# uf3/uf3

Hardware: AMD Instinct MI355X
Metric: featurized frames/sec (10k-atom, 2-elem, 2+3-body) (higher is better)
Workload: dtype f64

## Files before the change

### include/uf3_hip.h

```cpp
#ifndef UF3_HIP_H
#define UF3_HIP_H

#include <stddef.h>
#include <stdint.h>

#ifdef __cplusplus
extern "C" {
#endif

typedef struct uf3_ctx uf3_ctx;
typedef struct uf3_basis uf3_basis;

enum {
    UF3_OK = 0,
    UF3_EINVAL = 1,
    UF3_ESPECIES = 2,
    UF3_EHIP = 3,
    UF3_ENOMEM = 4,
    UF3_EOVERFLOW = 5,
    UF3_ERETRY = 6
};

typedef struct uf3_basis_spec {
    int32_t n_species;
// ... 35 lines not shown
int uf3_ctx_timing_read(uf3_ctx *ctx, double *featurize_ms, int64_t *featurize_launches,
                        double *neighbor_ms, double *gram_ms, double *eval_ms);

int uf3_ctx_md_skin(uf3_ctx *ctx, double skin);
int uf3_ctx_md_stats(uf3_ctx *ctx, int64_t *builds, int64_t *steps, int64_t *redone);

typedef struct uf3_fit uf3_fit;
int uf3_fit_create(uf3_basis *basis, int with_forces, int64_t max_atoms_per_chunk , const int64_t *frozen_idx,
                   const double *frozen_c, int32_t n_frozen, uf3_fit **out);
void uf3_fit_destroy(uf3_fit *fit);
int uf3_fit_reset(uf3_fit *fit);
int uf3_fit_add(uf3_fit *fit, int32_t n_frames, const int64_t *atom_counts, const double *const *positions, const void *const *z,
                int z_is_int64, const double *cells , const uint8_t *pbc , const double *energies,
                const double *const *forces );
int uf3_fit_pack(uf3_fit *fit, const int64_t *keep, int32_t n_keep, int allreduce, double *out_host);
int uf3_fit_info(const uf3_fit *fit, int64_t *n_chunks, double *n_energy_rows, double *n_force_rows);
int uf3_fit_use_flat(uf3_fit *fit, double *d_flat);
int uf3_fit_first_chunk(uf3_fit *fit, double fraction);

#define UF3_COMM_ID_BYTES 128
int uf3_comm_unique_id(uf3_ctx *ctx, void *id);
int uf3_comm_init(uf3_ctx *ctx, int n_ranks, int rank, const void *id);
int uf3_comm_destroy(uf3_ctx *ctx);
int uf3_comm_info(const uf3_ctx *ctx, int32_t *n_ranks, int32_t *rank);
int uf3_allreduce_sum_f64(uf3_ctx *ctx, double *d_buf, int64_t n);
int uf3_gram_allreduce(uf3_ctx *ctx, double *d_packed, int64_t n);

int uf3_basis_create(uf3_ctx *ctx, const uf3_basis_spec *spec, uf3_basis **out);
void uf3_basis_destroy(uf3_basis *basis);
int uf3_basis_featurizer_modes(const uf3_basis *basis, int32_t *mask);

int uf3_featurize(uf3_basis *basis, const uf3_frames *frames, const double *pos ,
                  const int32_t *z , double *x_e, double *x_f);
int uf3_featurize_dev(uf3_basis *basis, const uf3_frames *frames, const double *d_pos,
                      const int32_t *d_z, double *d_x_e, double *d_x_f);
int uf3_featurize_ld_dev(uf3_basis *basis, const uf3_frames *frames, const double *d_positions, const int32_t *d_z,
                         double *d_x_e, double *d_x_f, int64_t ld);

int uf3_gram(uf3_ctx *ctx, const double *x, const double *y, int64_t n_rows, int32_t n_feat,
             int64_t ld, int accumulate, double *gram, double *ord);
int uf3_gram_dev(uf3_ctx *ctx, const double *d_x, const double *d_y, int64_t n_rows,
                 int32_t n_feat, int64_t ld, int accumulate, double *d_gram, double *d_ord);
int uf3_gram_force_rows_dev(uf3_basis *basis, const double *d_x_f, const double *d_y_f, const int32_t *d_z,
                            int64_t n_atoms, int64_t ld, int accumulate, double *d_gram, double *d_ord);

int uf3_fit_rows_dev(uf3_ctx *ctx, int32_t n_frames, int32_t n_feat, double *d_x_e, const double *d_atom_counts,
                     const double *d_y_e, const double *d_y_f, int64_t n_y_f, const int64_t *d_frozen,
                     const double *d_c_frozen, int32_t n_frozen, double *d_moments );
int uf3_fit_pack_dev(uf3_ctx *ctx, int32_t n_feat, const double *d_flat, const int64_t *d_keep, int32_t n_keep,
                     const int64_t *d_frozen, const double *d_c_frozen, int32_t n_frozen, double n_energy_rows,
                     double n_force_rows, double *d_packed);

int uf3_eval(uf3_basis *basis, const uf3_frames *frames, const double *pos, const int32_t *z,
             const double *c1, const double *c2, const double *c3, double *energies, double *forces);
int uf3_eval_dev(uf3_basis *basis, const uf3_frames *frames, const double *d_pos, const int32_t *d_z,
                 const double *c1, const double *c2, const double *c3 ,
                 double *d_energies, double *d_forces);

int uf3_eval_virial(uf3_basis *basis, const uf3_frames *frames, const double *pos, const int32_t *z,
                    const double *c1, const double *c2, const double *c3, double *energies, double *forces,
                    double *virials);
int uf3_eval_virial_dev(uf3_basis *basis, const uf3_frames *frames, const double *d_pos, const int32_t *d_z,
                        const double *c1, const double *c2, const double *c3 ,
                        double *d_energies, double *d_forces, double *d_virials);

int uf3_eval_atoms(uf3_basis *basis, const uf3_frames *frames, const double *pos, const int32_t *z,
                   const double *c1, const double *c2, const double *c3, int64_t atom_begin, int64_t atom_end,
                   double *energies, double *forces, double *virials);
int uf3_eval_atoms_dev(uf3_basis *basis, const uf3_frames *frames, const double *d_pos, const int32_t *d_z,
                       const double *c1, const double *c2, const double *c3 , int64_t atom_begin,
                       int64_t atom_end, double *d_energies, double *d_forces, double *d_virials);

int uf3_eval_centres(uf3_basis *basis, const uf3_frames *frames, const double *pos, const int32_t *z,
                     const double *c1, const double *c2, const double *c3, int64_t atom_begin, int64_t atom_end,
                     double *energies, double *forces, double *virials);
int uf3_eval_centres_dev(uf3_basis *basis, const uf3_frames *frames, const double *d_pos, const int32_t *d_z,
                         const double *c1, const double *c2, const double *c3 , int64_t atom_begin,
                         int64_t atom_end, double *d_energies, double *d_forces, double *d_virials);

int uf3_neighbors_debug(uf3_basis *basis, const uf3_frames *frame, const double *pos, const int32_t *z,
                        int64_t *pair_count, int64_t *pair_ij, int64_t pair_cap,
                        int64_t *n3_count, int64_t *n3_ij, int64_t n3_cap);
int uf3_n3_lists_debug(uf3_basis *basis, int64_t natoms, int64_t *cap_out, int32_t *counts, int32_t *sidx, int64_t sidx_cap);

int uf3_pair_geometry(uf3_basis *basis, const uf3_frames *frame, const double *pos, const int32_t *z,
                      int64_t *pair_count, int64_t *pair_ij, double *pair_geo, int64_t pair_cap);

int uf3_pair_histogram(uf3_basis *basis, const uf3_frames *frames, const double *pos, const int32_t *z, int32_t n_bins,
                       const double *edges, int upper_inclusive, const double *noise, int64_t n_noise, int per_frame,
                       int64_t *out);
int uf3_pair_histogram_dev(uf3_basis *basis, const uf3_frames *frames, const double *d_pos, const int32_t *d_z, int32_t n_bins,
                           const double *edges, int upper_inclusive, const double *noise, int64_t n_noise, int per_frame,
                           int64_t *d_out);

int uf3_distance_matrix(uf3_ctx *ctx, const double *a, int64_t na, const double *b, int64_t nb, double *out);
int uf3_direction_cosines(uf3_ctx *ctx, const double *sup_pos, int64_t n_sup, const int64_t *i_where,
                          const int64_t *j_where, const double *rij, int64_t n_d, int64_t n_atoms, double *out);

#ifdef __cplusplus
}
#endif
#endif
```

### uf3_amd/_lib.py

```python
import ctypes as C
import sys
import importlib.util
import os
import threading
import weakref

import numpy as np

_HERE = os.path.dirname(os.path.abspath(__file__))
LIB_PATH = os.environ.get("UF3_LIB_PATH", os.path.join(_HERE, "csrc", "libuf3hip.so"))

EXPORTS = ["uf3_ctx_create", "uf3_ctx_destroy", "uf3_ctx_set_stream", "uf3_ctx_synchronize",
           "uf3_last_error", "uf3_build_id", "uf3_ctx_timing_reset", "uf3_ctx_timing_read",
           "uf3_ctx_use_own_stream", "uf3_basis_create", "uf3_basis_destroy", "uf3_basis_featurizer_modes",
           "uf3_featurize", "uf3_featurize_dev", "uf3_gram", "uf3_gram_dev",
           "uf3_eval", "uf3_eval_dev", "uf3_eval_virial", "uf3_eval_virial_dev", "uf3_eval_atoms", "uf3_eval_atoms_dev",
           "uf3_eval_centres", "uf3_eval_centres_dev",
           "uf3_neighbors_debug", "uf3_n3_lists_debug", "uf3_fit_rows_dev", "uf3_fit_pack_dev", "uf3_gram_force_rows_dev",
           "uf3_pair_geometry", "uf3_distance_matrix", "uf3_direction_cosines",
           "uf3_ctx_md_skin", "uf3_ctx_md_stats",
           "uf3_featurize_ld_dev", "uf3_fit_create", "uf3_fit_destroy", "uf3_fit_reset", "uf3_fit_add", "uf3_fit_pack", "uf3_fit_info", "uf3_fit_use_flat", "uf3_fit_first_chunk",
           "uf3_comm_unique_id", "uf3_comm_init", "uf3_comm_destroy", "uf3_comm_info", "uf3_allreduce_sum_f64", "uf3_gram_allreduce",
           "uf3_pair_histogram", "uf3_pair_histogram_dev"]


SOURCES = ("uf3_hip.hip", "uf3_kernels.h", "uf3_feat3.h", "uf3_device.h", os.path.join("..", "..", "include", "uf3_hip.h"))


def source_build_id(csrc_dir=None):
    import hashlib
    csrc_dir = csrc_dir or os.path.join(_HERE, "csrc")
    h = hashlib.sha256()
    for name in SOURCES:
        with open(os.path.join(csrc_dir, name), "rb") as f:
            h.update(f.read())
    return h.hexdigest()[:16]


def build_id():
    return load().uf3_build_id().decode()


class HipUnavailable(RuntimeError):
    pass


class UF3Error(RuntimeError):
    def __init__(self, code, message):
        super().__init__(f"libuf3hip error {code}: {message}")
        self.code = code


class SpeciesError(UF3Error):
    """A frame contains an element outside the basis (UF3_ESPECIES)."""


class RetryError(UF3Error):
    """UF3_ERETRY: an earlier asynchronous ``uf3_featurize_dev`` call overflowed its neighbour capacities (or met atoms
    far outside their cell, whose 3-body force rows need the launches with the reference's image-range rule); its outputs
    are invalid, the context has adapted: repeat the work since the last synchronisation."""


class BasisSpec(C.Structure):
    _fields_ = [("n_species", C.c_int32), ("species_z", C.c_void_p),
                ("n_pairs", C.c_int32), ("pair_z", C.c_void_p), ("pair_nk", C.c_void_p),
                ("pair_knots", C.c_void_p), ("pair_rmin", C.c_void_p), ("pair_rmax", C.c_void_p),
                ("pair_col", C.c_void_p), ("lead2", C.c_int32), ("trail2", C.c_int32),
                ("n_trios", C.c_int32), ("trio_z", C.c_void_p), ("trio_nk", C.c_void_p),
                ("trio_knots", C.c_void_p), ("trio_col", C.c_void_p), ("trio_ncol", C.c_void_p),
                ("trio_lut", C.c_void_p), ("n_feat", C.c_int32), ("r_cut", C.c_double)]


class Frames(C.Structure):
    _fields_ = [("n_frames", C.c_int32), ("atom_offsets", C.c_void_p), ("cells", C.c_void_p),
                ("pbc", C.c_void_p)]


_lib = None
_lock = threading.Lock()


def _share_hip_runtime_with_torch():
    if "torch" in sys.modules:
        return
    try:
        spec = importlib.util.find_spec("torch")
    except (ImportError, ValueError):
        return
    if spec is None or not spec.submodule_search_locations:
        return
    cand = os.path.join(list(spec.submodule_search_locations)[0], "lib", "libamdhip64.so")
    if os.path.exists(cand):
        try:
            C.CDLL(cand, mode=C.RTLD_GLOBAL)
        except OSError:
            pass


def load():
    global _lib
    with _lock:
        if _lib is not None:
            return _lib
        if not os.path.exists(LIB_PATH):
            raise HipUnavailable(
                f"{LIB_PATH} not found: build it with `make -C uf3_amd/csrc` "
                "(or `python -c 'import __graft_entry__ as g; g.build()'`). "
                "uf3_amd has no CPU fallback.")
        _share_hip_runtime_with_torch()
        lib = C.CDLL(LIB_PATH)
        vp, i32, i64, dbl = C.c_void_p, C.c_int32, C.c_int64, C.c_double
        lib.uf3_ctx_create.argtypes = [C.c_int, C.POINTER(vp)]
        lib.uf3_ctx_destroy.argtypes = [vp]
        lib.uf3_ctx_destroy.restype = None
        lib.uf3_ctx_set_stream.argtypes = [vp, vp]
        lib.uf3_ctx_use_own_stream.argtypes = [vp]
        lib.uf3_ctx_synchronize.argtypes = [vp]
        lib.uf3_last_error.argtypes = [vp]
        lib.uf3_last_error.restype = C.c_char_p
        lib.uf3_build_id.argtypes = []
        lib.uf3_build_id.restype = C.c_char_p
        lib.uf3_ctx_timing_reset.argtypes = [vp, C.c_int]
        lib.uf3_ctx_timing_read.argtypes = [vp, C.POINTER(dbl), C.POINTER(i64), C.POINTER(dbl),
                                            C.POINTER(dbl), C.POINTER(dbl)]
        lib.uf3_ctx_md_skin.argtypes = [vp, dbl]
        lib.uf3_fit_create.argtypes = [vp, C.c_int, i64, vp, vp, i32, C.POINTER(vp)]
        lib.uf3_fit_destroy.argtypes = [vp]
        lib.uf3_fit_destroy.restype = None
        lib.uf3_fit_reset.argtypes = [vp]
        lib.uf3_fit_add.argtypes = [vp, i32, vp, vp, vp, C.c_int, vp, vp, vp, vp]
        lib.uf3_fit_pack.argtypes = [vp, vp, i32, C.c_int, vp]
        lib.uf3_fit_info.argtypes = [vp, C.POINTER(i64), C.POINTER(dbl), C.POINTER(dbl)]
        lib.uf3_fit_use_flat.argtypes = [vp, vp]
        lib.uf3_fit_first_chunk.argtypes = [vp, dbl]
        lib.uf3_comm_unique_id.argtypes = [vp, vp]
        lib.uf3_comm_init.argtypes = [vp, C.c_int, C.c_int, vp]
        lib.uf3_comm_destroy.argtypes = [vp]
        lib.uf3_comm_info.argtypes = [vp, C.POINTER(i32), C.POINTER(i32)]
        lib.uf3_allreduce_sum_f64.argtypes = [vp, vp, i64]
        lib.uf3_gram_allreduce.argtypes = [vp, vp, i64]
        lib.uf3_ctx_md_stats.argtypes = [vp, C.POINTER(i64), C.POINTER(i64), C.POINTER(i64)]
        lib.uf3_basis_create.argtypes = [vp, C.POINTER(BasisSpec), C.POINTER(vp)]
        lib.uf3_basis_destroy.argtypes = [vp]
        lib.uf3_basis_destroy.restype = None
        lib.uf3_basis_featurizer_modes.argtypes = [vp, vp]
        for name in ("uf3_featurize", "uf3_featurize_dev"):
            getattr(lib, name).argtypes = [vp, C.POINTER(Frames), vp, vp, vp, vp]
        lib.uf3_featurize_ld_dev.argtypes = [vp, C.POINTER(Frames), vp, vp, vp, vp, i64]
        for name in ("uf3_gram", "uf3_gram_dev"):
            getattr(lib, name).argtypes = [vp, vp, vp, i64, i32, i64, C.c_int, vp, vp]
        for name in ("uf3_eval", "uf3_eval_dev"):
            getattr(lib, name).argtypes = [vp, C.POINTER(Frames), vp, vp, vp, vp, vp, vp, vp]
        for name in ("uf3_eval_virial", "uf3_eval_virial_dev"):
            getattr(lib, name).argtypes = [vp, C.POINTER(Frames), vp, vp, vp, vp, vp, vp, vp, vp]
        for name in ("uf3_eval_atoms", "uf3_eval_atoms_dev", "uf3_eval_centres", "uf3_eval_centres_dev"):
            getattr(lib, name).argtypes = [vp, C.POINTER(Frames), vp, vp, vp, vp, vp, i64, i64, vp, vp, vp]
        lib.uf3_neighbors_debug.argtypes = [vp, C.POINTER(Frames), vp, vp, vp, vp, i64, vp, vp, i64]
        lib.uf3_n3_lists_debug.argtypes = [vp, i64, vp, vp, vp, i64]
        lib.uf3_gram_force_rows_dev.argtypes = [vp, vp, vp, vp, i64, i64, i32, vp, vp]
        lib.uf3_pair_geometry.argtypes = [vp, C.POINTER(Frames), vp, vp, vp, vp, vp, i64]
        lib.uf3_distance_matrix.argtypes = [vp, vp, i64, vp, i64, vp]
        lib.uf3_direction_cosines.argtypes = [vp, vp, i64, vp, vp, vp, i64, i64, vp]
        lib.uf3_fit_rows_dev.argtypes = [vp, i32, i32, vp, vp, vp, vp, i64, vp, vp, i32, vp]
        lib.uf3_fit_pack_dev.argtypes = [vp, i32, vp, vp, i32, vp, vp, i32, dbl, dbl, vp]
        for name in ("uf3_pair_histogram", "uf3_pair_histogram_dev"):
            getattr(lib, name).argtypes = [vp, C.POINTER(Frames), vp, vp, i32, vp, C.c_int, vp, i64, C.c_int, vp]
        _lib = lib
        return lib


def _p(a):
    return None if a is None else a.ctypes.data_as(C.c_void_p)


def _addr(a):
    return None if a is None else a.__array_interface__["data"][0]


class Context:

    def __init__(self, device=0):
        self.lib = load()
        h = C.c_void_p()
        rc = self.lib.uf3_ctx_create(int(device), C.byref(h))
        if rc:
            msg = self.lib.uf3_last_error(None).decode()
            raise HipUnavailable(f"cannot create a HIP context on device {device}: {msg}")
        self.handle = h
        self.device = int(device)
        self._pid = os.getpid()

    def check(self, rc):
        if rc:
            msg = self.lib.uf3_last_error(self.handle).decode()
            raise {2: SpeciesError, 6: RetryError}.get(rc, UF3Error)(rc, msg)

    def set_stream(self, stream_ptr):
        prev = getattr(self, "_stream", None)
        self.check(self.lib.uf3_ctx_set_stream(self.handle, C.c_void_p(stream_ptr or 0)))
        self._stream = stream_ptr or 0
        return prev

    def use_own_stream(self):
        self.check(self.lib.uf3_ctx_use_own_stream(self.handle))
        self._stream = None

    def restore_stream(self, prev):
        if prev is None:
            self.use_own_stream()
        else:
            self.set_stream(prev)

    def synchronize(self):
        self.check(self.lib.uf3_ctx_synchronize(self.handle))

    def timing_reset(self, enable=True):
        self.check(self.lib.uf3_ctx_timing_reset(self.handle, int(enable)))

    def timing_read(self):
        f, n, nb, g, e = C.c_double(), C.c_int64(), C.c_double(), C.c_double(), C.c_double()
        self.check(self.lib.uf3_ctx_timing_read(self.handle, C.byref(f), C.byref(n), C.byref(nb),
                                                C.byref(g), C.byref(e)))
        return dict(featurize_ms=f.value, featurize_launches=n.value, neighbor_ms=nb.value,
                    gram_ms=g.value, eval_ms=e.value)

    def md_skin(self, skin):
        skin = float(skin)
        if getattr(self, "_md_skin", 0.0) != skin:
            self.check(self.lib.uf3_ctx_md_skin(self.handle, skin))
            self._md_skin = skin

    def comm_unique_id(self):
        buf = C.create_string_buffer(128)
        self.check(self.lib.uf3_comm_unique_id(self.handle, buf))
        return buf.raw

    def comm_init(self, n_ranks, rank, unique_id):
        self.check(self.lib.uf3_comm_init(self.handle, int(n_ranks), int(rank), C.c_char_p(bytes(unique_id))))

    def comm_destroy(self):
        self.check(self.lib.uf3_comm_destroy(self.handle))
# ... 269 lines not shown
```

### uf3_amd/csrc/uf3_device.h

```cpp
#pragma once
#include <hip/hip_runtime.h>
#include <stdint.h>
#include <type_traits>

#define UF3_MAX_SPECIES 8
#define UF3_MAX_PAIRS 36
#define WAVE 64

struct KnotRec {
    double t[6];
    double r[6];
};

struct LegDev {
    int rec_off;
    int nk;
    double t0, tlast;
    double inv_h;
};

struct PairDev {
    LegDev leg;
    int col;
    int nb;
// ... 12 lines not shown
    int dim_m, dim_n;
    int dim_l;
    int sc, sa, sb;
    int nsrc, src_off;
    int dense, lo[3], ext[3];
    double thr0, thr2;
    double gthr0, gthr2;
    int grouped;
    int banded;
    int band_tile[3];
    int layout;
    int gsrc_off;
    int wrow[3];
};

struct BasisDev {
    int S, P, T, F;
    int lead2, trail2;
    double rmin3, rmax3;
    double s3_lo, s3_hi;
    double rmax2;
    double rsearch;
    int trio_legs_uniform;
    int pairs_uniform;
    int pair_col[UF3_MAX_SPECIES * UF3_MAX_SPECIES];
    signed char z2s[120];
    short pair_of[UF3_MAX_SPECIES * UF3_MAX_SPECIES];
    short trio_of[UF3_MAX_SPECIES * UF3_MAX_SPECIES * UF3_MAX_SPECIES];
    PairDev pairs[UF3_MAX_PAIRS];
    const TrioDev *trios;
    const KnotRec *recs;
    const int *lut;
};

struct FrameGeom {
    double cell[9];
    double inv[9];
    double binw[3];
    int nb[3];
    int rad[3];
    int per[3];
    int fac[3];
    int cnt[3];
    double win_lo[3], win_hi[3];
    int bin_base;
    int atom_lo, atom_hi;
};

struct __attribute__((aligned(16))) SlotRec {
    double x, y, z;
    int atom;
    int ws;
};
__device__ __forceinline__ int pack_ws(int w0, int w1, int w2, int spec) {
    return (w0 + 256) | ((w1 + 256) << 9) | ((w2 + 256) << 18) | (spec << 27);
}
__device__ __forceinline__ void unpack_ws(int p, int &w0, int &w1, int &w2, int &spec) {
    w0 = (p & 511) - 256; w1 = ((p >> 9) & 511) - 256; w2 = ((p >> 18) & 511) - 256; spec = (p >> 27) & 15;
}

struct CellList {
    const int *bin_start;
    const SlotRec *slots;
    const int *atom_bin;
    const int *atom_wrap;
};

struct __attribute__((aligned(16))) N3Entry {
    double dx, dy, dz, r;
    int parent;
    int shiftc;
    int sidx;
    int spec;
};

struct N3Lists {
    int cap;
    int *cnt;
    int *spoff;
    N3Entry *ent;
    int xcap;
    int *xoff;
    N3Entry *xent;
};

__device__ __forceinline__ int pack3(int a, int b, int c) { return (a + 512) | ((b + 512) << 10) | ((c + 512) << 20); }
__device__ __forceinline__ void unpack3(int p, int &a, int &b, int &c) {
    a = (p & 1023) - 512; b = ((p >> 10) & 1023) - 512; c = ((p >> 20) & 1023) - 512;
}

__device__ __forceinline__ int image_pos(int s) { return s == 0 ? 0 : (s > 0 ? 2 * s - 1 : -2 * s); }

__device__ __forceinline__ int supercell_index(const FrameGeom &g, int s0, int s1, int s2, int local_atom) {
    int rank = (image_pos(s1) * g.cnt[0] + image_pos(s0)) * g.cnt[2] + image_pos(s2);
    return rank * (g.atom_hi - g.atom_lo) + local_atom;
}

__device__ __forceinline__ int find_interval(const KnotRec *recs, const LegDev &leg, double x) {
    int hi = leg.nk - 5;
    int i = 3 + (int)((x - leg.t0) * leg.inv_h);
    i = i < 3 ? 3 : (i > hi ? hi : i);
    const KnotRec *base = recs + leg.rec_off;
    for (;;) {
        double ti = base[i].t[2], ti1 = base[i].t[3];
        if (x > ti1 && i < hi) ++i;
        else if (x <= ti && i > 3) --i;
        else break;
    }
    return i;
}

typedef double __attribute__((ext_vector_type(2))) KnotPair;
template <int AS> struct KnotPairs { typedef const KnotPair *type; };
template <> struct KnotPairs<1> { typedef const __attribute__((address_space(1))) KnotPair *type; };
template <> struct KnotPairs<3> { typedef const __attribute__((address_space(3))) KnotPair *type; };

template <int AS = 0>
__device__ __forceinline__ void load_knot_rec(const KnotRec *p, KnotRec &k) {
    typename KnotPairs<AS>::type q = (typename KnotPairs<AS>::type)(const KnotPair *)p;
    const KnotPair v0 = q[0], v1 = q[1], v2 = q[2], v3 = q[3], v4 = q[4], v5 = q[5];
    __builtin_amdgcn_sched_group_barrier(0x120, 6, 0);
    k.t[0] = v0.x; k.t[1] = v0.y; k.t[2] = v1.x; k.t[3] = v1.y; k.t[4] = v2.x; k.t[5] = v2.y;
    k.r[0] = v3.x; k.r[1] = v3.y; k.r[2] = v4.x; k.r[3] = v4.y; k.r[4] = v5.x; k.r[5] = v5.y;
}

template <int AS = 0>
__device__ __forceinline__ int load_interval(const KnotRec *recs, const LegDev &leg, double x, KnotRec &k) {
    const int hi = leg.nk - 5;
    int i = 3 + (int)((x - leg.t0) * leg.inv_h);
    i = i < 3 ? 3 : (i > hi ? hi : i);
    const KnotRec *base = recs + leg.rec_off;
    load_knot_rec<AS>(base + i, k);
    if (__builtin_expect(x > k.t[3] && i < hi, 0)) {
        do { ++i; load_knot_rec<AS>(base + i, k); } while (x > k.t[3] && i < hi);
    } else if (__builtin_expect(x <= k.t[2] && i > 3, 0)) {
        do { --i; load_knot_rec<AS>(base + i, k); } while (x <= k.t[2] && i > 3);
    }
    return i;
}

template <int AS = 0>
__device__ __forceinline__ int load_interval_guess(const KnotRec *recs, const LegDev &leg, double x, KnotRec &k) {
    const int hi = leg.nk - 5;
    int i = 3 + (int)((x - leg.t0) * leg.inv_h);
    i = i < 3 ? 3 : (i > hi ? hi : i);
    load_knot_rec<AS>(recs + leg.rec_off + i, k);
    return i;
}
template <int AS = 0>
__device__ __forceinline__ int load_interval_fix(const KnotRec *recs, const LegDev &leg, double x, int i, KnotRec &k) {
    const int hi = leg.nk - 5;
    const KnotRec *base = recs + leg.rec_off;
    if (__builtin_expect(x > k.t[3] && i < hi, 0)) {
        do { ++i; load_knot_rec<AS>(base + i, k); } while (x > k.t[3] && i < hi);
    } else if (__builtin_expect(x <= k.t[2] && i > 3, 0)) {
        do { --i; load_knot_rec<AS>(base + i, k); } while (x <= k.t[2] && i > 3);
    }
    return i;
}

template <bool DERIV>
__device__ __forceinline__ void bspline4(const KnotRec &k, double x, double *v, double *d) {
    double l1 = x - k.t[2], l2 = x - k.t[1], l3 = x - k.t[0];
    double r1 = k.t[3] - x, r2 = k.t[4] - x, r3 = k.t[5] - x;
    double tmp = k.r[0];
    double n0 = r1 * tmp, n1 = l1 * tmp;
// ... 63 lines not shown
}
__device__ __forceinline__ int mbcnt(unsigned long long mask) {
    return __builtin_amdgcn_mbcnt_hi((unsigned)(mask >> 32), __builtin_amdgcn_mbcnt_lo((unsigned)mask, 0));
}

template <class F>
__device__ __forceinline__ void for_each_candidate(const FrameGeom &g, const CellList &cl, int m, F f, int range_mult = 1) {
    const int lane = lane_id();
    const int lb = cl.atom_bin[m];
    const int b2 = lb % g.nb[2], b1 = (lb / g.nb[2]) % g.nb[1], b0 = lb / (g.nb[2] * g.nb[1]);
    int w0, w1, w2;
    unpack3(cl.atom_wrap[m], w0, w1, w2);
    int lo[3], hi[3];
    for (int k = 0; k < 3; k++) {
        if (g.per[k]) { lo[k] = -g.rad[k]; hi[k] = g.rad[k]; }
        else if (g.nb[k] == 1) { lo[k] = 0; hi[k] = 0; }
        else if (g.nb[k] == 2) { lo[k] = 0; hi[k] = 1; }
        else { lo[k] = -1; hi[k] = 1; }
    }
    auto fdiv = [](int t, int n) { return t >= 0 ? t / n : -((n - 1 - t) / n); };
    const int n1 = hi[1] - lo[1] + 1, n01 = (hi[0] - lo[0] + 1) * n1;
    const int sh2_lo = fdiv(b2 + lo[2], g.nb[2]), nr2 = fdiv(b2 + hi[2], g.nb[2]) - sh2_lo + 1;
    const int n_runs = n01 * nr2;
    for (int r0 = 0; r0 < n_runs; r0 += WAVE) {
        const int r = r0 + lane;
        int len = 0, slot0 = 0, shp = 0;
        if (r < n_runs) {
            const int i01 = r / nr2, q = r - i01 * nr2, i0 = i01 / n1, i1 = i01 - i0 * n1;
            const int t0 = b0 + lo[0] + i0, t1 = b1 + lo[1] + i1;
            int sh0 = fdiv(t0, g.nb[0]), sh1 = fdiv(t1, g.nb[1]), sh2 = sh2_lo + q;
            const int c0 = t0 - sh0 * g.nb[0], c1 = t1 - sh1 * g.nb[1];
            const int o2a = max(lo[2], sh2 * g.nb[2] - b2), o2b = min(hi[2], (sh2 + 1) * g.nb[2] - 1 - b2);
            const int c2 = b2 + o2a - sh2 * g.nb[2];
            if (!g.per[0]) sh0 = 0;
            if (!g.per[1]) sh1 = 0;
            if (!g.per[2]) sh2 = 0;
            const int gb = g.bin_base + (c0 * g.nb[1] + c1) * g.nb[2] + c2;
            slot0 = cl.bin_start[gb];
            len = cl.bin_start[gb + (o2b - o2a + 1)] - slot0;
            shp = pack3(sh0, sh1, sh2);
        }
        const int incl = wave_scan_incl(len);
        const int total = __builtin_amdgcn_readlane(incl, WAVE - 1);
        const int rel = slot0 - (incl - len);
        const unsigned long long nonempty = __ballot(len > 0);
        const unsigned long long behind = lane < WAVE - 1 ? nonempty >> (lane + 1) : 0ull;
        const int next_ne = behind ? lane + 1 + __builtin_ctzll(behind) : WAVE;
        auto fetch = [&](int wbase, SlotRec &sr, int &shpk) {
            const int idx = wbase + lane;
            const int p = incl - wbase;
            const bool sender = (len > 0) & (p > 0) & (p < WAVE);
            const int got = __builtin_amdgcn_ds_permute((sender ? p : 0) << 2, sender ? next_ne + 1 : 0);
            const unsigned long long holds = __ballot((len > 0) & (p > 0));
            const int first = holds ? __builtin_ctzll(holds) : 0;
            const int reached = wave_scan_max(lane == 0 ? 0 : got);
            const int run = min(reached ? reached - 1 : first, WAVE - 1);
            const int slot = __shfl(rel, run) + idx;
            shpk = __shfl(shp, run);
            sr = cl.slots[idx < total ? slot : 0];
        };
        SlotRec sr_next;
        int shp_next;
        if (total > 0) fetch(0, sr_next, shp_next);
        for (int base = 0; base < total; base += WAVE) {
            const int idx = base + lane;
            SlotRec sr = sr_next;
            const int shpk = shp_next;
            if (base + WAVE < total) fetch(base + WAVE, sr_next, shp_next);
            int sh0, sh1, sh2;
            unpack3(shpk, sh0, sh1, sh2);
            bool ok = idx < total;
            int s0 = 0, s1 = 0, s2 = 0, sj = 0;
            if (ok) {
                int v0, v1, v2;
                unpack_ws(sr.ws, v0, v1, v2, sj);
                s0 = sh0 - v0 + w0; s1 = sh1 - v1 + w1; s2 = sh2 - v2 + w2;
                ok = (abs(s0) <= range_mult * g.fac[0]) && (abs(s1) <= range_mult * g.fac[1]) && (abs(s2) <= range_mult * g.fac[2]);
                if (ok && sr.atom == m && s0 == 0 && s1 == 0 && s2 == 0) ok = false;
            } else { sr.x = sr.y = sr.z = 0.0; sr.atom = 0; sr.ws = 0; }
            f(ok, sr, sj, s0, s1, s2);
        }
    }
}
```

### uf3_amd/csrc/uf3_feat3.h

```cpp
#pragma once

struct Feat3Leg {
    double t0, tlast, inv_h;
    int nk, row0;
};

struct Feat3Args {
    const BasisDev *B;
    const TrioDev *trios;
    const double *rows;
    int n_rows;
    const unsigned short *fsrc;
    const int *trio_fsrc;
    int n_fsrc;
    Feat3Leg leg_p, leg_n;
    int lo_p, ext_p, lo_n, ext_n;
    int pr_rows;
    const FrameGeom *geoms;
    const int *frame_of;
    N3Lists n3;
    const double *pos;
    const signed char *spec;
    double *x_e, *x_f;
    int ld;
    int natoms, atoms_per_block, e_direct;
    const int *sel;
    int sel_mode, sel_cap;
    int skip;
    double *wbuf;
    int wsz;
    int m_lo;
};

template <int EF, int NR>
struct F3Cfg {
    static constexpr int PS = 32 * NR;
    static constexpr int EFP = (EF + 1) & ~1;
    static constexpr int RS_N = EFP + 16 + (NR == 1 ? 2 : 0);
    static constexpr int RS_C = NR == 1 ? 10 : (NR == 2 ? 12 : 14);
    static constexpr int NREC = NR == 1 ? 29 : 32;
    static constexpr int DUMP = NR == 1 ? 4 * EF * 32 : 2 * (EF * PS + 2);
    static constexpr int STAGE0 = 64 * RS_C > NREC * RS_N ? 64 * RS_C : NREC * RS_N;
    static constexpr int STAGE = (STAGE0 > DUMP ? STAGE0 : DUMP) + 4;
    static constexpr int MIN_WAVES = NR == 1 ? 4 : 2;
};

typedef double __attribute__((ext_vector_type(2))) F3Pair;
typedef const __attribute__((address_space(3))) F3Pair *F3LdsPairs;
typedef const __attribute__((address_space(3))) double *F3LdsDoubles;

#ifndef F3_ROWS_GLOBAL
#define F3_ROWS_GLOBAL 0
#endif
typedef const __attribute__((address_space(1))) F3Pair *F3GlobalPairs;
template <bool DERIV>
__device__ __forceinline__ int f3_eval(const double *rows, const Feat3Leg &lg, double x, double (&v)[4], double (&d)[4]) {
    const int hi = lg.nk - 5;
    int iv = 3 + (int)((x - lg.t0) * lg.inv_h);
    iv = iv < 3 ? 3 : (iv > hi ? hi : iv);
    F3Pair kn, cf[8];
    auto load_row = [&](int i) {
#if F3_ROWS_GLOBAL
        F3GlobalPairs q = (F3GlobalPairs)(const F3Pair *)(rows + (size_t)(lg.row0 + i - 3) * 18);
#else
        F3LdsPairs q = (F3LdsPairs)(const F3Pair *)(rows + (size_t)(lg.row0 + i - 3) * 18);
#endif
        F3Pair t0 = q[0], t[8];
#pragma unroll
        for (int e = 0; e < 8; e++) t[e] = q[1 + e];
        kn = t0;
#pragma unroll
        for (int e = 0; e < 8; e++) cf[e] = t[e];
        __builtin_amdgcn_sched_group_barrier(F3_ROWS_GLOBAL ? 0x020 : 0x100, 9, 0);
    };
    load_row(iv);
    if (__builtin_expect(x > kn.y && iv < hi, 0)) {
        do { ++iv; load_row(iv); } while (x > kn.y && iv < hi);
    } else if (__builtin_expect(x <= kn.x && iv > 3, 0)) {
        do { --iv; load_row(iv); } while (x <= kn.x && iv > 3);
    }
    const double u = x - kn.x;
#pragma unroll
    for (int fq = 0; fq < 4; fq++) {
        const double c0 = cf[2 * fq].x, c1 = cf[2 * fq].y, c2 = cf[2 * fq + 1].x, c3 = cf[2 * fq + 1].y;
        double pv = fma(c3, u, c2), pd = fma(c3, u, pv);
        pv = fma(pv, u, c1); pd = fma(pd, u, pv);
        pv = fma(pv, u, c0);
        v[fq] = pv;
        if (DERIV) d[fq] = pd;
    }
    return iv;
}

#ifndef F3_WIDE_MINW
#define F3_WIDE_MINW 2
#endif
template <bool WANT_E, int EF, int NR, int CAP = 0, bool HO = false>
__global__ void __launch_bounds__(WPB * WAVE, (NR == 1 ? 4 : F3_WIDE_MINW))
k_featurize3(Feat3Args A) {
    static_assert(!HO || NR == 1, "the hand-off buffer is laid out for the one-round window");
    typedef F3Cfg<EF, NR> Cfg;
    constexpr int RS_C = Cfg::RS_C, RS_N = Cfg::RS_N, NREC = Cfg::NREC, PS = Cfg::PS, EFP = Cfg::EFP;
    extern __shared__ __align__(16) unsigned char smem[];
    const BasisDev *B = A.B;
    const int F = load_const(&B->F), S = load_const(&B->S), n_trios = load_const(&B->T), cap = CAP > 0 ? CAP : A.n3.cap;
    const int ent_stride = A.n3.cap;
    if (A.sel_mode) {
        const int seen = load_const(A.sel);
        if ((seen <= A.sel_cap) != (A.sel_mode == 1)) return;
    }
    const int tid = threadIdx.x, lane = tid & 63;
    const int wave = __builtin_amdgcn_readfirstlane(tid >> 6);
    double *erow = (double *)smem;
    const bool e_lds = WANT_E && !A.e_direct;
    const size_t e_d = e_lds ? (size_t)F + (F & 1) : 0;
    double *rows_lds = erow + e_d;
    const double *rows = F3_ROWS_GLOBAL ? A.rows : rows_lds;
    const size_t rows_d = (size_t)A.n_rows * 18;
    const size_t list_d = 5 * (size_t)cap + ((5 * cap) & 1), tq_d = (size_t)cap * EF * 4;
    constexpr size_t stage_d = Cfg::STAGE;
    const size_t per_wave_d = list_d + tq_d + stage_d;
    const size_t per_wave_i = 2 * (size_t)cap + 2 * ((size_t)cap + 1) + (UF3_MAX_SPECIES + 2) + (size_t)cap * (S + 1) + 2 * NREC + cap;
    double *wd = rows_lds + rows_d + (size_t)wave * per_wave_d;
    int *wi = (int *)(rows_lds + rows_d + (size_t)WPB * per_wave_d) + (size_t)wave * per_wave_i;
    double *ox = wd, *oy = ox + cap, *oz = oy + cap, *orr = oz + cap, *oir = orr + cap;
    double *tq = wd + list_d;
    double *stage = tq + tq_d;
    double *zq = stage + (Cfg::STAGE - 4);
    int *oparent = wi, *oshift = wi + cap, *noff = wi + 2 * cap, *nbase = noff + cap + 1, *so = nbase + cap + 1;
    int *osbp = so + (UF3_MAX_SPECIES + 2);
    int *hdrs = osbp + cap;
    int *ospoff = hdrs + 2 * NREC;
    const int sp_stride = S + 1;
    unsigned short *fsrc_l = (unsigned short *)((int *)(rows_lds + rows_d + (size_t)WPB * per_wave_d) + (((size_t)WPB * per_wave_i + 3) & ~(size_t)3));

    for (int q = tid; q < (int)rows_d; q += WPB * WAVE) rows_lds[q] = A.rows[q];
    for (int q = tid; q < A.n_fsrc / 2; q += WPB * WAVE) ((int *)fsrc_l)[q] = ((const int *)A.fsrc)[q];
    if (e_lds) { for (int q = tid; q < F; q += WPB * WAVE) erow[q] = 0.0; }
    for (int q = lane; q < (int)stage_d; q += WAVE) stage[q] = 0.0;
    for (int q = lane; q < (int)tq_d; q += WAVE) tq[q] = 0.0;
    __syncthreads();

    const int ext_p = A.ext_p, ext_n = A.ext_n, lo_n = A.lo_n, lo_p = A.lo_p, npos = ext_p * ext_n;
    const int half = lane >> 5;
    int p_lane[NR], n_lane[NR], qn_lane[NR], n32_lane[NR];
    const int pr_rows = A.pr_rows;
#pragma unroll
    for (int r = 0; r < NR; r++) {
        const int pl = (lane & 31) / ext_n, p = r * pr_rows + pl;
        const bool on = pl < pr_rows && p < ext_p;
        p_lane[r] = on ? p : 0;
        n_lane[r] = on ? (lane & 31) - pl * ext_n : -(1 << 20);
        qn_lane[r] = on ? n_lane[r] : RS_C - 1;
        n32_lane[r] = n_lane[r] * 32;
    }
    (void)npos;
    const int sbn_max = ext_n > 4 ? ext_n - 4 : 0, sbp_max = ext_p > 4 ? ext_p - 4 : 0;
    const Feat3Leg leg_p = A.leg_p, leg_n = A.leg_n;
    auto rounds_of = [&](int sb) {
        if (EF <= 4) return (1 << NR) - 1;
        const int r0 = sb / pr_rows, r1 = min(sb + 3, ext_p - 1) / pr_rows;
        return ((2 << r1) - 1) & ~((1 << r0) - 1);
    };

    const int bid = (blockIdx.x & 7) * (gridDim.x >> 3) + (blockIdx.x >> 3);
    const int block_first = A.m_lo + bid * A.atoms_per_block;
    const int block_end = min(block_first + A.atoms_per_block, A.natoms);
    int erow_frame = -1;
    for (int m0 = block_first; m0 < block_end; m0 += WPB) {
        const int m = m0 + wave;
        const bool active = m < block_end;
        if (e_lds) {
            int f_first = load_const(A.frame_of + m0);
            if (f_first != erow_frame) {
                __syncthreads();
                if (erow_frame >= 0)
                    for (int q = tid; q < F; q += WPB * WAVE) {
                        double v = erow[q];
                        if (v != 0.0) { unsafeAtomicAdd(A.x_e + (size_t)erow_frame * F + q, v); erow[q] = 0.0; }
                    }
                __syncthreads();
                erow_frame = f_first;
            }
        }
        if (!active) continue;
        const int fr = load_const(A.frame_of + m);
        const int sm = ((const __attribute__((address_space(4))) signed char *)(unsigned long long)A.spec)[m];
        ESink es;
        es.lds = erow; es.glob = WANT_E ? A.x_e + (size_t)fr * F : nullptr; es.direct = !e_lds || (fr != erow_frame);

        const int n_own = load_const(A.n3.cnt + m);
        wave_sync();
        for (int e = lane; e < n_own; e += WAVE) {
            const N3Entry en = A.n3.ent[(size_t)m * ent_stride + e];
            ox[e] = en.dx; oy[e] = en.dy; oz[e] = en.dz; orr[e] = en.r; oir[e] = 1.0 / en.r;
            int s0, s1, s2;
            unpack3(en.shiftc, s0, s1, s2);
            oparent[e] = en.parent; oshift[e] = pack3(-s0, -s1, -s2);
        }
        if (lane <= S) so[lane] = A.n3.spoff[(size_t)m * (UF3_MAX_SPECIES + 1) + lane];
        wave_sync();
        if (!HO)
            for (int e = lane; e < n_own; e += WAVE) {
                const int *src = A.n3.spoff + (size_t)oparent[e] * (UF3_MAX_SPECIES + 1);
                for (int sp = 0; sp <= S; sp++) ospoff[e * (S + 1) + sp] = src[sp];
            }
        for (int e = lane; e < n_own; e += WAVE) {
            const double r = orr[e];
            double v[4] = {0, 0, 0, 0}, d[4] = {0, 0, 0, 0};
            int sbp = 0;
            if (r > leg_p.t0 && r < leg_p.tlast && !UF3_SKIP(32)) {
                const int iv = f3_eval<true>(rows, leg_p, r, v, d);
                sbp = max(0, min(sbp_max, iv - 3 - lo_p));
            }
            if (EF > 4) osbp[e] = sbp;
            const double ir = oir[e], ux = ox[e] * ir, uy = oy[e] * ir, uz = oz[e] * ir;
            double *dst = tq + (size_t)e * EF * 4;
            if (EF > 4) {
#pragma unroll
                for (int q = 0; q < EF; q++) { *(double2 *)(dst + 4 * q) = double2{0.0, 0.0}; *(double2 *)(dst + 4 * q + 2) = double2{0.0, 0.0}; }
                dst += 4 * sbp;
            }
#pragma unroll
            for (int q = 0; q < (EF < 4 ? EF : 4); q++) {
                *(double2 *)(dst + 4 * q) = double2{ux * d[q], uy * d[q]};
                *(double2 *)(dst + 4 * q + 2) = double2{uz * d[q], v[q]};
            }
        }
        wave_sync();

        for (int t = 0; t < n_trios; t++) {
            const TrioDev *td = A.trios + t;
            typedef int int8_v __attribute__((ext_vector_type(8)));
            const int8_v hv = *(const __attribute__((address_space(4))) int8_v *)(unsigned long long)&td->head;
            const int t_ncol = hv[2], t_sc = hv[3], t_sa = hv[4], t_sb = hv[5], t_col = hv[6];
            const bool centre = t_sc == sm, nbr = t_sa == sm || t_sb == sm;
            if (!centre && !nbr) { zero_rows(A.x_f, m, A.ld, t_col, t_ncol); continue; }
            const bool tr = t_sa != t_sb && sm == t_sb;

            double xacc[NR][EF][2], ws[NR][2];
#pragma unroll
            for (int r = 0; r < NR; r++) {
                ws[r][0] = ws[r][1] = 0.0;
#pragma unroll
                for (int q = 0; q < EF; q++) { xacc[r][q][0] = xacc[r][q][1] = 0.0; }
            }
            int cur = -1;

            int wmask = 0;
            auto flush = [&](bool is_c) {
                if (cur < 0 || UF3_SKIP(2)) return;
                const double *tc = tq + (size_t)cur * EF * 4;
                F3Pair tv[EF];
                double t3[EF];
#pragma unroll
                for (int q = 0; q < EF; q++) {
                    tv[q] = *(F3LdsPairs)(const F3Pair *)(tc + 4 * q + 2 * half); t3[q] = ((F3LdsDoubles)tc)[4 * q + 3];
                }
#pragma unroll
                for (int r = 0; r < NR; r++) {
                    if (EF > 4 && !((wmask >> r) & 1)) continue;
                    const int lo = __double2loint(ws[r][1]), hi = __double2hiint(ws[r][1]);
                    const auto r0 = __builtin_amdgcn_permlane32_swap(lo, lo, false, false);
                    const auto r1 = __builtin_amdgcn_permlane32_swap(hi, hi, false, false);
                    const double wpl = __hiloint2double(r1[1], r0[1]);
                    const double wpl1 = (half && !is_c) ? 0.0 : wpl, ws1 = half ? 0.0 : ws[r][1];
#pragma unroll
                    for (int q = 0; q < EF; q++) {
                        xacc[r][q][0] = fma(tv[q].x, wpl, fma(t3[q], ws[r][0], xacc[r][q][0]));
                        xacc[r][q][1] = fma(tv[q].y, wpl1, fma(t3[q], ws1, xacc[r][q][1]));
                    }
                    ws[r][0] = ws[r][1] = 0.0;
                }
                wmask = 0;
            };

            if (centre && !UF3_SKIP(4)) {
                const int fs = tr ? t_sb : t_sa, gs = tr ? t_sa : t_sb;
                const int f_lo = so[fs], nF = so[fs + 1] - f_lo, g_lo = so[gs], nG = so[gs + 1] - g_lo;
                const bool same = t_sa == t_sb;
                const int total = __builtin_amdgcn_readfirstlane(nF * nG);
                const int nGs = __builtin_amdgcn_readfirstlane(nG), f_los = __builtin_amdgcn_readfirstlane(f_lo),
                          g_los = __builtin_amdgcn_readfirstlane(g_lo);
                const float rcp_ng = __builtin_amdgcn_rcpf((float)max(nG, 1));
                for (int p0 = 0; p0 < total; p0 += WAVE) {
                    const int p = p0 + lane;
                    bool valid = p < total;
                    int fi = (int)(((float)p + 0.5f) * rcp_ng);
                    fi -= (fi * nG > p) ? 1 : 0;
                    fi += ((fi + 1) * nG <= p) ? 1 : 0;
                    const int gi = p - fi * nG;
                    valid = valid && (!same || gi > fi);
                    const int f = f_lo + fi, gg = g_lo + gi;
                    double bn[4] = {0, 0, 0, 0}, dum[4];
                    int sbn = 0;
                    if (valid) {
                        const double rf = orr[f], rg = orr[gg];
                        const double ex = ox[gg] - ox[f], ey = oy[gg] - oy[f], ez = oz[gg] - oz[f];
                        const double rn = norm3_leg(ex, ey, ez);
                        valid = (rf > leg_p.t0) & (rf < leg_p.tlast) & (rg > leg_p.t0) & (rg < leg_p.tlast) &
                                (rn > leg_n.t0) & (rn < leg_n.tlast);
                        if (valid && !UF3_SKIP(64)) {
                            const int iv = f3_eval<false>(rows, leg_n, rn, bn, dum);
                            sbn = max(0, min(sbn_max, iv - 3 - lo_n));
                        }
                    }
                    int smask = (1 << NR) - 1;
                    if (EF > 4) {
                        const int rm = valid ? rounds_of(osbp[gg]) : 0;
                        smask = 0;
#pragma unroll
                        for (int r = 0; r < NR; r++) smask |= __ballot((rm >> r) & 1) ? (1 << r) : 0;
                    }
                    {
                        double *rp = stage + (size_t)lane * RS_C;
#pragma unroll
                        for (int u = 0; u < RS_C; u += 2) *(double2 *)(rp + u) = double2{0.0, 0.0};
                        if (valid) {
#pragma unroll
                            for (int u = 0; u < 4; u++) rp[sbn + u] = bn[u];
                        }
                    }
                    wave_sync();
                    const int p1 = min(total, p0 + WAVE);
                    int fi_s = p0 / nGs;
                    for (int pr = fi_s * nGs; pr < p1 && !UF3_SKIP(1); pr += nGs, fi_s++) {
                        int s0 = max(pr, p0), s1 = min(pr + nGs, p1);
                        if (same) s0 = max(s0, pr + fi_s + 1);
                        if (s0 >= s1) continue;
                        const int key = f_los + fi_s;
                        if (key != cur) { flush(true); cur = key; }
                        wmask |= smask;
                        const double *qp = stage + (size_t)(s0 - p0) * RS_C;
                        const double *tp = tq + (size_t)(g_los + (s0 - pr)) * EF * 4 + 2 * half;
                        int cnt = s1 - s0;
                        auto body = [&](auto tag) {
                            constexpr int CNT = decltype(tag)::value;
#pragma unroll
                            for (int r = 0; r < NR; r++) {
                                if (EF > 4 && !((smask >> r) & 1)) continue;
                                double bq[CNT];
                                F3Pair tt[CNT];
#pragma unroll
                                for (int i = 0; i < CNT; i++) {
                                    bq[i] = ((F3LdsDoubles)qp)[i * RS_C + qn_lane[r]];
                                    tt[i] = *(F3LdsPairs)(const F3Pair *)(tp + (size_t)i * EF * 4 + 4 * p_lane[r]);
                                }
#pragma unroll
                                for (int i = 0; i < CNT; i++) { ws[r][0] = fma(tt[i].x, bq[i], ws[r][0]); ws[r][1] = fma(tt[i].y, bq[i], ws[r][1]); }
                            }
                            qp += CNT * RS_C; tp += (size_t)CNT * EF * 4; cnt -= CNT;
                        };
                        while (cnt >= 4) body(std::integral_constant<int, 4>{});
                        if (cnt == 3) body(std::integral_constant<int, 3>{});
                        else if (cnt == 2) body(std::integral_constant<int, 2>{});
                        else if (cnt == 1) body(std::integral_constant<int, 1>{});
                    }
                    wave_sync();
                }
                flush(true);
                cur = -1;
            }
            if (HO && nbr && !UF3_SKIP(8)) {
                const int sx = sm == t_sa ? t_sb : t_sa;
                const int rc_lo = __builtin_amdgcn_readfirstlane(so[t_sc]), ncen = __builtin_amdgcn_readfirstlane(so[t_sc + 1]) - rc_lo;
                const bool lane_on = n_lane[0] >= 0;
                const size_t wstep = (size_t)S * A.wsz;
                const double *wb = A.wbuf + (((size_t)(m - A.m_lo) * ent_stride + rc_lo) * S + sx) * A.wsz + (lane & 31) * 4 + 2 * half;
                for (int e0 = 0; e0 < ncen; e0 += 4) {
                    F3Pair w[4];
#pragma unroll
                    for (int i = 0; i < 4; i++) {
                        const int idx = min(e0 + i, ncen - 1);
                        w[i] = lane_on ? __builtin_nontemporal_load((const F3Pair *)(wb + (size_t)idx * wstep)) : F3Pair{0.0, 0.0};
                    }
#pragma unroll
                    for (int i = 0; i < 4; i++)
                        if (e0 + i < ncen) {
                            cur = rc_lo + e0 + i;
                            ws[0][0] = w[i].x; ws[0][1] = w[i].y;
                            flush(false);
                        }
                }
                cur = -1;
            }
            if (!HO && nbr && !UF3_SKIP(8)) {
                const int sx = sm == t_sa ? t_sb : t_sa;
                const int rc_lo = so[t_sc], ncen = so[t_sc + 1] - rc_lo;
                int total_n = 0;
                for (int e0 = 0; e0 < ncen; e0 += WAVE) {
                    const int e = e0 + lane;
                    int cnt = 0, base = 0;
                    if (e < ncen) {
                        const int *sp = ospoff + (size_t)(rc_lo + e) * sp_stride;
                        base = sp[sx]; cnt = sp[sx + 1] - base;
                    }
                    const int incl = wave_scan_incl(cnt);
                    if (e < ncen) { noff[e] = total_n + incl - cnt; nbase[e] = base; }
                    total_n += __builtin_amdgcn_readlane(incl, WAVE - 1);
                }
                total_n = __builtin_amdgcn_readfirstlane(total_n);
                if (lane == 0) noff[ncen] = total_n;
                wave_sync();
                for (int p0 = 0; p0 < total_n; p0 += WAVE) {
                    const int q = p0 + lane;
                    bool valid = q < total_n;
                    double pv[4] = {0, 0, 0, 0}, bn[4] = {0, 0, 0, 0}, bd[4] = {0, 0, 0, 0}, a3[3] = {0, 0, 0}, dum[4];
                    int sbn = 0, sbp = 0, e = 0;
                    if (valid) {
                        int lo = 0, hi = ncen - 1;
                        while (lo < hi) { const int mid = (lo + hi + 1) >> 1; if (noff[mid] <= q) lo = mid; else hi = mid - 1; }
                        e = rc_lo + lo;
                        const int kk = nbase[lo] + (q - noff[lo]);
                        const int pc = oparent[e];
                        const double oex = ox[e], oey = oy[e], oez = oz[e], oer = orr[e];
                        const N3Entry ke = A.n3.ent[(size_t)pc * ent_stride + kk];
                        valid = !(ke.parent == m && ke.shiftc == oshift[e]);
                        const double ex = oex + ke.dx, ey = oey + ke.dy, ez = oez + ke.dz;
                        const double rn = norm3_leg(ex, ey, ez), rk = ke.r;
                        valid = valid & (oer > leg_p.t0) & (oer < leg_p.tlast) & (rk > leg_p.t0) & (rk < leg_p.tlast) &
                                (rn > leg_n.t0) & (rn < leg_n.tlast);
                        if (valid && !UF3_SKIP(64)) {
                            const double in = fast_rcp(rn);
                            a3[0] = ex * in; a3[1] = ey * in; a3[2] = ez * in;
                            const int ivp = f3_eval<false>(rows, leg_p, rk, pv, dum);
                            sbp = max(0, min(sbp_max, ivp - 3 - lo_p));
                            const int iv = f3_eval<true>(rows, leg_n, rn, bn, bd);
                            sbn = max(0, min(sbn_max, iv - 3 - lo_n));
                        }
                    }
                    const unsigned long long mask = __ballot(valid);
                    const int nv = __popcll(mask), rank = mbcnt(mask);
                    int smask = (1 << NR) - 1;
                    if (EF > 4) {
                        const int rm = valid ? rounds_of(sbp) : 0;
                        smask = 0;
#pragma unroll
                        for (int r = 0; r < NR; r++) smask |= __ballot((rm >> r) & 1) ? (1 << r) : 0;
                    }
                    for (int sp0 = 0; sp0 < nv; sp0 += NREC) {
                        const int slot = rank - sp0;
                        if (valid && slot >= 0 && slot < NREC) {
                            double *rp = stage + (size_t)slot * RS_N;
                            if (EF > 4) {
#pragma unroll
                                for (int u = 0; u < EFP; u += 2) *(double2 *)(rp + u) = double2{0.0, 0.0};
#pragma unroll
                                for (int u = 0; u < 4; u++) rp[sbp + u] = pv[u];
                            } else {
                                *(double2 *)rp = double2{pv[0], pv[1]};
                                *(double2 *)(rp + 2) = double2{pv[2], pv[3]};
                            }
#pragma unroll
                            for (int u = 0; u < 4; u++) {
                                *(double2 *)(rp + EFP + 4 * u) = double2{a3[0] * bd[u], a3[1] * bd[u]};
                                *(double2 *)(rp + EFP + 2 + 4 * u) = double2{a3[2] * bd[u], bn[u]};
                            }
                            hdrs[slot] = e; hdrs[NREC + slot] = sbn * 32;
                        }
                        wave_sync();
                        const int r_end = min(NREC, nv - sp0);
                        const int v_key = hdrs[min(lane, NREC - 1)], v_prev = hdrs[min(max(lane - 1, 0), NREC - 1)];
                        unsigned long long gm = __ballot(lane < r_end && (lane == 0 || v_key != v_prev));
                        while (gm && !UF3_SKIP(1)) {
                            const int g0 = __builtin_ctzll(gm);
                            gm &= gm - 1;
                            const int g1 = gm ? __builtin_ctzll(gm) : r_end;
                            const int key = __builtin_amdgcn_readlane(v_key, g0);
                            if (key != cur) { flush(false); cur = key; }
                            wmask |= smask;
                            const double *rp = stage + (size_t)g0 * RS_N;
                            const int *sp = hdrs + NREC + g0;
                            int cnt = g1 - g0;
                            auto body = [&](auto tag) {
                                constexpr int CNT = decltype(tag)::value;
                                int sb[CNT];
#pragma unroll
                                for (int i = 0; i < CNT; i++) sb[i] = ((const __attribute__((address_space(3))) int *)sp)[i];
#pragma unroll
                                for (int r = 0; r < NR; r++) {
                                    if (EF > 4 && !((smask >> r) & 1)) continue;
                                    double bq[CNT];
                                    F3Pair tt[CNT];
#pragma unroll
                                    for (int i = 0; i < CNT; i++) {
                                        const unsigned off = (unsigned)(n32_lane[r] - sb[i]);
                                        const char *qa = (const char *)(rp + i * RS_N + EFP + 2 * half) + off;
                                        qa = off < 128u ? qa : (const char *)zq;
                                        bq[i] = ((F3LdsDoubles)rp)[i * RS_N + p_lane[r]];
                                        tt[i] = *(F3LdsPairs)(const F3Pair *)qa;
                                    }
#pragma unroll
                                    for (int i = 0; i < CNT; i++) { ws[r][0] = fma(bq[i], tt[i].x, ws[r][0]); ws[r][1] = fma(bq[i], tt[i].y, ws[r][1]); }
                                }
                                rp += CNT * RS_N; sp += CNT; cnt -= CNT;
                            };
                            while (cnt >= 4) body(std::integral_constant<int, 4>{});
                            if (cnt == 3) body(std::integral_constant<int, 3>{});
                            else if (cnt == 2) body(std::integral_constant<int, 2>{});
                            else if (cnt == 1) body(std::integral_constant<int, 1>{});
                        }
                        wave_sync();
                    }
                }
                flush(false);
                cur = -1;
            }
            if (UF3_SKIP(16)) continue;
            wave_sync();
            const unsigned short *ft = fsrc_l + load_const(A.trio_fsrc + t) + (size_t)(tr ? 2 * t_ncol : 0);
            if (NR == 1) {
#pragma unroll
                for (int q = 0; q < EF; q++)
                    *(double2 *)(stage + (size_t)(((half * EF + q) * 32 + (lane & 31)) * 2)) = double2{xacc[0][q][0], xacc[0][q][1]};
                wave_sync();
                for (int col = lane; col < t_ncol; col += WAVE) {
                    const int s0 = ft[2 * col], s1 = ft[2 * col + 1];
                    F3LdsPairs d0 = (F3LdsPairs)(const F3Pair *)stage, d1 = d0 + EF * 32;
                    const F3Pair a0 = d0[s0], a1 = d0[s1], b0 = d1[s0], b1 = d1[s1];
                    double *dst = A.x_f + (size_t)m * 3 * A.ld + t_col + col;
                    __builtin_nontemporal_store(a0.x + a1.x, dst); __builtin_nontemporal_store(a0.y + a1.y, dst + A.ld);
                    __builtin_nontemporal_store(b0.x + b1.x, dst + 2 * (size_t)A.ld);
                    if (WANT_E) es.add(t_col + col, b0.y + b1.y);
                }
                wave_sync();
            } else {
                constexpr int BUF = EF * PS + 2;
#pragma unroll
                for (int k = 0; k < 2; k++) {
#pragma unroll
                    for (int r = 0; r < NR; r++)
#pragma unroll
                        for (int q = 0; q < EF; q++) stage[half * BUF + q * PS + r * 32 + (lane & 31)] = xacc[r][q][k];
                    if (lane == 0 || lane == 32) stage[half * BUF + EF * PS] = 0.0;
                    wave_sync();
                    for (int col = lane; col < t_ncol; col += WAVE) {
                        const int s0 = ft[2 * col], s1 = ft[2 * col + 1];
                        F3LdsDoubles da = (F3LdsDoubles)stage, db = da + BUF;
                        const double va = da[s0] + da[s1];
                        __builtin_nontemporal_store(va, A.x_f + ((size_t)m * 3 + k) * A.ld + t_col + col);
                        if (k == 0 || WANT_E) {
                            const double vb = db[s0] + db[s1];
                            if (k == 0) __builtin_nontemporal_store(vb, A.x_f + ((size_t)m * 3 + 2) * A.ld + t_col + col);
                            else es.add(t_col + col, vb);
                        }
                    }
                    wave_sync();
                }
            }
        }
    }
    if (e_lds) {
        __syncthreads();
        if (erow_frame >= 0)
            for (int q = tid; q < F; q += WPB * WAVE) {
                double v = erow[q];
                if (v != 0.0) unsafeAtomicAdd(A.x_e + (size_t)erow_frame * F + q, v);
            }
    }
}

#ifndef F3W_NRECP
#define F3W_NRECP 32
#endif
struct F3WCfg {
    static constexpr int RS_W = 38;
    static constexpr int NRECP = F3W_NRECP;
    static constexpr int STAGE = NRECP * RS_W;
};

template <int EF, int CAP = 0>
__global__ void __launch_bounds__(WPB * WAVE, 4)
k_feat3_w(Feat3Args A) {
    static_assert(EF <= 4, "one-round windows only");
    constexpr int RS_W = F3WCfg::RS_W, NRECP = F3WCfg::NRECP;
    extern __shared__ __align__(16) unsigned char smem[];
    const BasisDev *B = A.B;
    const int S = load_const(&B->S), n_trios = load_const(&B->T), cap = CAP > 0 ? CAP : A.n3.cap;
    const int ent_stride = A.n3.cap;
    if (A.sel_mode) {
        const int seen = load_const(A.sel);
        if ((seen <= A.sel_cap) != (A.sel_mode == 1)) return;
    }
    const int tid = threadIdx.x, lane = tid & 63;
    const int wave = __builtin_amdgcn_readfirstlane(tid >> 6);
// ... 165 lines not shown
```

### uf3_amd/csrc/uf3_hip.hip

```cpp
#include <algorithm>
#include <cmath>
#include <cstdio>
#include <cstring>
#include <map>
#include <mutex>
#include <string>
#include <vector>
#include <thread>

#include <hip/hip_runtime.h>
#include <rocprim/rocprim.hpp>

#include "../../include/uf3_hip.h"
#include "uf3_kernels.h"
#include "uf3_feat3.h"
#include <chrono>
#include <dlfcn.h>

struct Buf {
    void *p = nullptr;
    size_t cap = 0;
    bool fine = false;
    hipError_t ensure(size_t bytes) {
        if (bytes <= cap) return hipSuccess;
        if (p) { hipError_t e = hipFree(p); if (e != hipSuccess) return e; p = nullptr; cap = 0; }
        fine = false;
        size_t want = bytes + bytes / 4 + 256;
        hipError_t e = hipMalloc(&p, want);
        if (e == hipSuccess) cap = want;
        return e;
    }
    hipError_t ensure_fine(size_t bytes) {
        if (bytes <= cap && fine) return hipSuccess;
        if (p) { hipError_t e = hipFree(p); if (e != hipSuccess) return e; p = nullptr; cap = 0; }
        fine = false;
        size_t want = std::max(bytes, cap) + bytes / 4 + 256;
        hipError_t e = hipExtMallocWithFlags(&p, want, hipDeviceMallocFinegrained);
        if (e == hipSuccess) { cap = want; fine = true; }
        return e;
    }
    void release() { if (p) hipFree(p); p = nullptr; cap = 0; }
    template <class T> T *as() const { return (T *)p; }
};

struct PinBuf {
    void *p = nullptr;
    size_t cap = 0;
    hipError_t ensure(size_t bytes) {
        if (bytes <= cap) return hipSuccess;
        if (p) hipHostFree(p);
        p = nullptr; cap = 0;
        size_t want = std::max(bytes, (size_t)4096);
        hipError_t e = hipHostMalloc(&p, want, hipHostMallocCoherent);
        if (e == hipSuccess) cap = want;
        return e;
    }
    void release() { if (p) hipHostFree(p); p = nullptr; cap = 0; }
};
#define UF3_PIN_LIMIT (512 * 1024)
#define UF3_BAR_LIMIT (128 * 1024)

struct uf3_ctx {
    int device = 0;
    hipStream_t own_stream = nullptr, stream = nullptr;
    std::string err;
    int lds_max = 65536;
    int n_cu = 256;
    Buf geoms, offsets, frame_of, atom_bin, atom_wrap, spec, key_in, key_out, val_in, val_out, sort_tmp,
        bin_start, slots, flags,
        n3_cnt, n3_int, n3_dbl, e_atom, nbr_f, coeff, stage_pos, stage_z, stage_out, stage_out2,
        gram_tiles[UF3_MAX_SPECIES + 1], gram_tij, frag, dbg,
        sp_rows, sp_seg,
        halo,
        n3x_ent, n3x_off,
        bin_cnt,
        part_sums,
        hist_edges, hist_noise,
        f3w;
    int n3_cap = 0, cand_cap = 0;
    size_t bin_cnt_clean = 0;
    int n3_last_cap = 0, n3_last_natoms = 0;
    int n3x_cap = 0;
    bool img_mode = false;
    int gram_plan_np[UF3_MAX_SPECIES + 1] = {0}, gram_plan_blocks[UF3_MAX_SPECIES + 1] = {0}, gram_plan_next = 0;
    int gram_direct_feat = 0;
    bool n3_tuned = false;
    bool cand_tuned = false;
    struct Pending { hipEvent_t ev = nullptr; int cap = 0, cand = 0, xcap = 0; bool has3 = false, img = true, img_launch = false, live = false; };
    enum { N_PENDING = 16 };
    Pending pending_chk[N_PENDING];
    PinBuf pin_flags;
    int pending_head = 0;
    int async_bad = 0;
    std::string async_msg;
    bool frag_ready = false;
    int32_t *d_stage_z = nullptr;
    bool bar_ok = false;
    bool bar_tested = false;
    Buf stage_bar;
    char *stage_cur = nullptr;
    size_t staged_in_dev = 0;
    bool env_no_feat3 = false, env_f3_no_cap16 = false, env_f3_no_select = false, env_debug_lds = false;
    int env_f3_bps = 24;
    unsigned eval_seq = 0;
    bool tail_signalled = false;
    bool pin_in_busy = false;
    size_t pin_in_pending = 0;
    PinBuf pin_in, pin_geo, pin_out;
    PinBuf pin_eval;
    hipEvent_t pin_in_done = nullptr, pin_geo_done = nullptr;
    std::vector<double> coeff_shadow;
    Buf coeff_cw;
    const void *cw_of = nullptr;
    const void *coeff_dev = nullptr;
    struct MdState {
        bool cap_tuned = false;
        bool verify_next = false;
        bool flags_clean = false;
        double skin = 0.0;
        bool valid = false;
        bool stale = false;
        const uf3_basis *basis = nullptr;
        int natoms = 0, n_frames = 0, cap = 0;
        std::vector<int64_t> offsets;
        std::vector<double> cells;
        std::vector<uint8_t> pbc;
        Buf ent, cnt, pos_ref, geo, frame_of, spec;
        Buf inbox, surv, mark;
        size_t inbox_zeroed = 0;
        size_t geo_bytes = 0;
        long long builds = 0, steps = 0, redone = 0;
    } md;
    void *comm = nullptr;
    int comm_ranks = 0, comm_rank = -1;
    bool md_step = false;
    bool timing = false;
    hipEvent_t ev0 = nullptr, ev1 = nullptr;
    double t_feat = 0, t_nbr = 0, t_gram = 0, t_eval = 0;
    long long n_feat_launch = 0;
    std::vector<std::pair<hipEvent_t, hipEvent_t>> pending[4];
};

struct uf3_basis {
    uf3_ctx *ctx = nullptr;
    BasisDev host;
    BasisDev *dev = nullptr;
    TrioDev *d_trios = nullptr;
    KnotRec *d_recs = nullptr;
    int *d_lut = nullptr;
    int *d_colsrc = nullptr;
    int *d_dsrc = nullptr;
    unsigned short *d_gsrc = nullptr;
    size_t n_gsrc = 0;
    bool all_grouped7 = false;
    bool all_banded9 = false;
    size_t n_dsrc = 0;
    int *d_sp_cols = nullptr;
    int sp_ncols[UF3_MAX_SPECIES] = {0};
    std::vector<int> block_bounds;
    size_t c2_len = 0, c3_len = 0, n_recs = 0;
    size_t n_pair_recs = 0;
    size_t trio_rec_lo = 0;
    size_t wrow_lo = 0;
    int n_wrows = 0;
// ... 34 lines not shown
        if (eq) g_env.vars.emplace_back(std::string(*e, eq - *e), std::string(eq + 1));
    }
}
static const char *uf3_env(const char *name) {
    if (g_env.print == ~0ull) uf3_env_refresh();
    for (const auto &kv : g_env.vars)
        if (kv.first == name) return kv.second.c_str();
    return nullptr;
}

static inline void uf3_store_fence() {
#if defined(__x86_64__) || defined(__i386__)
    __builtin_ia32_sfence();
#else
    __sync_synchronize();
#endif
}

static thread_local std::string g_err;
static int fail(uf3_ctx *ctx, int code, const std::string &msg) {
    if (ctx) ctx->err = msg;
    g_err = msg;
    return code;
}
#define HIPCHK(ctx, call)                                                                         \
    do {                                                                                          \
        hipError_t e__ = (call);                                                                  \
        if (e__ != hipSuccess)                                                                    \
            return fail(ctx, UF3_EHIP, std::string(#call) + ": " + hipGetErrorString(e__));       \
    } while (0)

extern "C" const char *uf3_last_error(const uf3_ctx *ctx) { return ctx ? ctx->err.c_str() : g_err.c_str(); }
#ifndef UF3_BUILD_ID
#define UF3_BUILD_ID "unknown"
#endif
extern "C" const char *uf3_build_id(void) { return UF3_BUILD_ID; }

static void read_f3_env(uf3_ctx *c) {
    c->env_no_feat3 = uf3_env("UF3_NO_FEAT3") != nullptr;
    c->env_f3_no_cap16 = uf3_env("UF3_F3_NO_CAP16") != nullptr;
    c->env_f3_no_select = uf3_env("UF3_F3_NO_SELECT") != nullptr;
    c->env_debug_lds = uf3_env("UF3_DEBUG_LDS") != nullptr;
    c->env_f3_bps = uf3_env("UF3_F3_BPS") ? std::max(1, atoi(uf3_env("UF3_F3_BPS"))) : 24;
}

extern "C" int uf3_ctx_create(int device, uf3_ctx **out) {
    uf3_env_refresh();
    if (!out) return fail(nullptr, UF3_EINVAL, "uf3_ctx_create: null out");
    int n = 0;
    hipError_t e = hipGetDeviceCount(&n);
    if (e != hipSuccess || n <= 0)
        return fail(nullptr, UF3_EHIP, std::string("no HIP device available: ") + hipGetErrorString(e));
    if (device < 0 || device >= n) return fail(nullptr, UF3_EINVAL, "uf3_ctx_create: bad device index");
    uf3_ctx *c = new uf3_ctx();
    c->device = device;
    HIPCHK(c, hipSetDevice(device));
    HIPCHK(c, hipStreamCreateWithFlags(&c->own_stream, hipStreamNonBlocking));
    c->stream = c->own_stream;
    HIPCHK(c, hipEventCreateWithFlags(&c->pin_in_done, hipEventDisableTiming));
    HIPCHK(c, hipEventCreateWithFlags(&c->pin_geo_done, hipEventDisableTiming));
    hipDeviceProp_t prop;
    HIPCHK(c, hipGetDeviceProperties(&prop, device));
    c->lds_max = (int)prop.sharedMemPerBlock;
    c->n_cu = prop.multiProcessorCount;
    read_f3_env(c);
    { int large = 0; c->bar_ok = hipDeviceGetAttribute(&large, hipDeviceAttributeIsLargeBar, device) == hipSuccess && large && !uf3_env("UF3_NO_BAR_STAGE"); }
    if (std::string(prop.gcnArchName).find("gfx950") == std::string::npos) {
        std::string m = std::string("uf3_hip is built for gfx950 only, device is ") + prop.gcnArchName;
        delete c;
        return fail(nullptr, UF3_EHIP, m);
    }
    *out = c;
    return UF3_OK;
}

extern "C" int uf3_comm_destroy(uf3_ctx *c);
extern "C" void uf3_ctx_destroy(uf3_ctx *c) {
    if (!c) return;
    hipSetDevice(c->device);
    hipStreamSynchronize(c->stream);
    Buf *all[] = {&c->geoms, &c->offsets, &c->frame_of, &c->atom_bin, &c->atom_wrap, &c->spec, &c->key_in,
                  &c->key_out, &c->val_in, &c->val_out, &c->sort_tmp, &c->bin_start, &c->slots, &c->flags, &c->n3_cnt, &c->n3_int, &c->n3_dbl, &c->e_atom, &c->nbr_f, &c->coeff,
                  &c->stage_pos, &c->stage_z, &c->stage_out, &c->stage_out2, &c->sp_rows, &c->sp_seg, &c->gram_tij, &c->frag, &c->dbg, &c->halo, &c->n3x_ent, &c->n3x_off,
                  &c->bin_cnt, &c->f3w, &c->coeff_cw, &c->part_sums};
    for (Buf *b : all) b->release();
    for (Buf &b : c->gram_tiles) b.release();
    if (c->comm) uf3_comm_destroy(c);
    { Buf *mdb[] = {&c->md.ent, &c->md.cnt, &c->md.pos_ref, &c->md.geo, &c->md.frame_of, &c->md.spec, &c->md.inbox, &c->md.surv, &c->md.mark}; for (Buf *b : mdb) b->release(); }
    c->stage_bar.release();
    c->pin_in.release(); c->pin_geo.release(); c->pin_out.release(); c->pin_flags.release(); c->pin_eval.release();
    for (auto &pd : c->pending_chk) if (pd.ev) hipEventDestroy(pd.ev);
    if (c->pin_in_done) hipEventDestroy(c->pin_in_done);
    if (c->pin_geo_done) hipEventDestroy(c->pin_geo_done);
    for (auto &v : c->pending) for (auto &p : v) { hipEventDestroy(p.first); hipEventDestroy(p.second); }
    if (c->own_stream) hipStreamDestroy(c->own_stream);
    delete c;
}

extern "C" int uf3_ctx_set_stream(uf3_ctx *c, void *s) {
    if (!c) return fail(nullptr, UF3_EINVAL, "null ctx");
    c->stream = (hipStream_t)s;
    return UF3_OK;
}

extern "C" int uf3_ctx_use_own_stream(uf3_ctx *c) {
    if (!c) return fail(nullptr, UF3_EINVAL, "null ctx");
    c->stream = c->own_stream;
    return UF3_OK;
}

static int check_flags(uf3_ctx *c);
static int poll_pending(uf3_ctx *c, bool wait, bool remember = true);

extern "C" int uf3_ctx_synchronize(uf3_ctx *c) {
    if (!c) return fail(nullptr, UF3_EINVAL, "null ctx");
    HIPCHK(c, hipSetDevice(c->device));
    HIPCHK(c, hipStreamSynchronize(c->stream));
    poll_pending(c, true);
    if (c->async_bad) {
        const int rc = c->async_bad;
        const std::string msg = c->async_msg;
        c->async_bad = 0; c->async_msg.clear();
        return fail(c, rc, msg);
    }
    return check_flags(c);
}

static int sync_own_call(uf3_ctx *c) {
    HIPCHK(c, hipStreamSynchronize(c->stream));
    int rc = poll_pending(c, true, false);
    if (rc) return rc;
    return check_flags(c);
}

enum { T_FEAT = 0, T_NBR = 1, T_GRAM = 2, T_EVAL = 3 };
struct Timed {
    uf3_ctx *c; int cls; hipEvent_t a = nullptr, b = nullptr;
    Timed(uf3_ctx *c_, int cls_) : c(c_), cls(cls_) {
        if (c->timing) { hipEventCreate(&a); hipEventCreate(&b); hipEventRecord(a, c->stream); }
    }
    ~Timed() {
        if (c->timing) { hipEventRecord(b, c->stream); c->pending[cls].push_back({a, b}); if (cls == T_FEAT) c->n_feat_launch++; }
    }
};

extern "C" int uf3_ctx_timing_reset(uf3_ctx *c, int enable) {
    if (!c) return fail(nullptr, UF3_EINVAL, "null ctx");
    hipStreamSynchronize(c->stream);
    for (auto &v : c->pending) { for (auto &p : v) { hipEventDestroy(p.first); hipEventDestroy(p.second); } v.clear(); }
    c->t_feat = c->t_nbr = c->t_gram = c->t_eval = 0;
    c->n_feat_launch = 0;
    c->timing = enable != 0;
    return UF3_OK;
}

extern "C" int uf3_ctx_timing_read(uf3_ctx *c, double *feat_ms, int64_t *feat_launches, double *nbr_ms,
                                   double *gram_ms, double *eval_ms) {
    if (!c) return fail(nullptr, UF3_EINVAL, "null ctx");
    HIPCHK(c, hipStreamSynchronize(c->stream));
    double *acc[4] = {&c->t_feat, &c->t_nbr, &c->t_gram, &c->t_eval};
    for (int k = 0; k < 4; k++) {
        for (auto &p : c->pending[k]) {
            float ms = 0;
            hipEventElapsedTime(&ms, p.first, p.second);
            *acc[k] += ms;
            hipEventDestroy(p.first); hipEventDestroy(p.second);
        }
// ... 622 lines not shown
    for (int k = 0; k < 3; k++) {
        double h = vol / norm3(nrm[k]);
        g.cnt[k] = g.per[k] ? 2 * g.fac[k] + 1 : 1;
        if (g.per[k]) {
            int nb = (int)std::floor(h / (rs * bin_frac));
            nb = std::max(1, std::min(nb, 256));
            g.nb[k] = nb;
            g.rad[k] = (int)std::ceil(rs / (h / nb) - 1e-12);
            if (g.rad[k] < 1) g.rad[k] = 1;
            g.binw[k] = 1.0 / nb;
            if (g.fac[k] > 400) return fail(c, UF3_EINVAL, "cell is too small relative to the cutoff");
            const double w = g.fac[k] + 1.0 - b->r_cut / h - 1e-9;
            g.win_lo[k] = 0.5 - 0.5 * w; g.win_hi[k] = 0.5 + 0.5 * w;
        } else {
            g.win_lo[k] = -1e300; g.win_hi[k] = 1e300;
            g.nb[k] = nb_np;
            g.rad[k] = 1;
            g.binw[k] = rs / h;
        }
        nbins *= g.nb[k];
    }
    long long m = (long long)g.cnt[0] * g.cnt[1] * g.cnt[2] * n;
    if (m >= (1LL << 31)) return fail(c, UF3_EINVAL, "reference supercell index exceeds int32");
    g.bin_base = bin_cursor;
    if (nbins + bin_cursor >= (1LL << 30)) return fail(c, UF3_EINVAL, "too many cell-list bins");
    bin_cursor += (int)nbins;
    return UF3_OK;
}

struct Prepared {
    int natoms = 0, n_frames = 0, nbins = 0;
    double max_density = 0;
    CellList cl;
    N3Lists n3;
    const FrameGeom *geoms = nullptr;
    const int *frame_of = nullptr;
    const signed char *spec = nullptr;
    const int64_t *d_offsets = nullptr;
    size_t geo_bytes = 0;
    bool deferred = false;
    bool flags_zeroed = false;
    bool small_prepared = false;
};

static int check_flags(uf3_ctx *c) {
    if (!c->flags.p) return UF3_OK;
    int fl[4] = {0, 0, 0, 0};
    HIPCHK(c, hipMemcpy(fl, c->flags.p, sizeof(fl), hipMemcpyDeviceToHost));
    if (fl[0] == 2) { hipMemset(c->flags.p, 0, sizeof(fl)); return fail(c, UF3_ESPECIES, "frame contains an element outside the basis"); }
    if (fl[0] == 1) { hipMemset(c->flags.p, 0, sizeof(fl)); return fail(c, UF3_EINVAL, "atom too far outside the periodic cell (|wrap| > 250)"); }
    return UF3_OK;
}

static int poll_pending(uf3_ctx *c, bool wait, bool remember) {
    int rc = UF3_OK;
    for (int q = 0; q < uf3_ctx::N_PENDING; q++) {
        uf3_ctx::Pending &p = c->pending_chk[(c->pending_head + q) % uf3_ctx::N_PENDING];
        if (!p.live) continue;
        if (wait) { HIPCHK(c, hipEventSynchronize(p.ev)); }
        else if (hipEventQuery(p.ev) != hipSuccess) continue;
        p.live = false;
        const int *fl = (const int *)c->pin_flags.p + 8 * ((c->pending_head + q) % uf3_ctx::N_PENDING);
        if (fl[0] == 2 && !rc) rc = fail(c, UF3_ESPECIES, "frame contains an element outside the basis (earlier asynchronous call)");
        else if (fl[0] == 1 && !rc) rc = fail(c, UF3_EINVAL, "atom too far outside the periodic cell (|wrap| > 250) (earlier asynchronous call)");
        bool grown = false;
        if (p.has3 && fl[1] > p.cap) { c->n3_cap = std::max(c->n3_cap, (std::max(fl[1] + 8, p.cap + p.cap / 4) + 7) / 8 * 8); grown = true; }
        if (fl[2] > p.cand) { c->cand_cap = std::max(c->cand_cap, (std::max(fl[2] + 16, p.cand + p.cand / 4) + 7) / 8 * 8); grown = true; }
        if (fl[3] > p.xcap) { c->n3x_cap = std::max(c->n3x_cap, std::min(248, (fl[3] + 8 + 7) / 8 * 8)); grown = true; }
        if (fl[4] && !p.img) { c->img_mode = true; grown = true; }
        else if (!fl[4] && p.img_launch) c->img_mode = false;
        if (grown && !rc)
            rc = fail(c, UF3_ERETRY, "an earlier asynchronous featurizer call overflowed its neighbour capacities: its outputs are "
                                     "invalid; the capacities have been raised, repeat the work since the last synchronisation");
    }
    if (rc && c->flags.p) hipMemsetAsync(c->flags.p, 0, sizeof(int), c->stream);
    if (rc && remember && !c->async_bad) { c->async_bad = rc; c->async_msg = c->err; }
    return rc;
}

static int n3_alloc(uf3_ctx *c, int natoms, int cap, N3Lists &n3) {
    HIPCHK(c, c->n3_cnt.ensure(sizeof(int) * (size_t)natoms * (UF3_MAX_SPECIES + 2)));
    HIPCHK(c, c->n3_dbl.ensure(sizeof(N3Entry) * (size_t)natoms * cap));
    n3.cap = cap;
    c->n3_last_cap = cap; c->n3_last_natoms = natoms;
    n3.cnt = c->n3_cnt.as<int>();
    n3.spoff = n3.cnt + natoms;
    n3.ent = c->n3_dbl.as<N3Entry>();
    return UF3_OK;
}

static int n3_cap_estimate(const uf3_basis *b, double dens) {
    double r = b->host.rmax3;
    double est = dens > 0 ? 4.18879 * r * r * r * dens : 24.0;
    return std::max(16, ((int)(est * 1.8) + 8 + 7) / 8 * 8);
}

static int n3_tune(uf3_ctx *c, const N3Lists &n3, int natoms) {
    hipStream_t st = c->stream;
    int *flags = c->flags.as<int>();
    c->n3_tuned = true;
    HIPCHK(c, hipMemsetAsync(flags + 6, 0, sizeof(int), st));
    hipLaunchKernelGGL(k_max_count, dim3(64), dim3(256), 0, st, n3.cnt, natoms, flags + 6);
    int seen = 0;
    HIPCHK(c, hipMemcpyAsync(&seen, flags + 6, sizeof(int), hipMemcpyDeviceToHost, st));
    HIPCHK(c, hipStreamSynchronize(st));
    c->n3_cap = std::max(8, (seen + 7) / 8 * 8);
    return UF3_OK;
}

static int build_halo_lists(uf3_basis *b, const Prepared &P, const N3Lists &n3, const double *d_pos, int lo, int hi,
                            bool marks_zeroed = false) {
    uf3_ctx *c = b->ctx;
    hipStream_t st = c->stream;
    const int natoms = P.natoms, nb_ = hi - lo;
    HIPCHK(c, c->halo.ensure(sizeof(int) * ((size_t)natoms + 4)));
    int *mark = c->halo.as<int>(), *range = mark + natoms;
    if (!marks_zeroed) HIPCHK(c, hipMemsetAsync(mark, 0, sizeof(int) * (size_t)natoms, st));
    if (nb_ <= 0 || natoms - nb_ <= 0) return UF3_OK;
    const size_t lds = (size_t)n3.cap * (8 + 32 + 16);
    hipLaunchKernelGGL(k_mark_halo, dim3((nb_ + 3) / 4), dim3(256), 0, st, n3, lo, hi, mark, range);
    hipLaunchKernelGGL(k_build_n3, dim3(natoms - nb_), dim3(64), lds, st, b->dev, P.geoms, P.frame_of, P.cl, n3, d_pos,
                       natoms, c->flags.as<int>() + 1, 0, (const int *)mark, (const int *)range);
    HIPCHK(c, hipGetLastError());
    return UF3_OK;
}

static int prepare(uf3_basis *b, const uf3_frames *fr, const double *d_pos, const int32_t *d_z, bool need_n3,
                   Prepared &P, bool defer_check = false, int64_t n3_lo = 0, int64_t n3_hi = -1, double extra_radius = 0.0) {
    uf3_ctx *c = b->ctx;
    c->md.flags_clean = false;
    if (!fr || fr->n_frames < 1 || !fr->atom_offsets || !fr->cells || !fr->pbc)
        return fail(c, UF3_EINVAL, "bad uf3_frames");
    if (fr->atom_offsets[0] != 0) return fail(c, UF3_EINVAL, "atom_offsets[0] must be 0");
    int nf = fr->n_frames;
    int64_t total = fr->atom_offsets[nf];
    if (total < 1 || total >= (1LL << 31) / 8) return fail(c, UF3_EINVAL, "batch must hold 1 .. 2^28 atoms");
    for (int f = 0; f < nf; f++)
        if (fr->atom_offsets[f + 1] < fr->atom_offsets[f]) return fail(c, UF3_EINVAL, "atom_offsets must be non-decreasing");
    int natoms = (int)total;
    std::vector<FrameGeom> geoms(nf);
    int bin_cursor = 0;
    double dens = 0;
    for (int f = 0; f < nf; f++) {
        int rc = make_geom(c, b, fr, f, geoms[f], bin_cursor, extra_radius);
        if (rc) return rc;
        int n = geoms[f].atom_hi - geoms[f].atom_lo;
        double vol = 0;
        if (geoms[f].per[0] && geoms[f].per[1] && geoms[f].per[2]) {
            double cr[3];
            cross3(geoms[f].cell + 3, geoms[f].cell + 6, cr);
            vol = std::fabs(dot3(geoms[f].cell, cr));
        }
        if (vol > 0) dens = std::max(dens, n / vol);
    }
    int nbins = bin_cursor;
    hipStream_t st = c->stream;
    HIPCHK(c, hipSetDevice(c->device));
    const size_t geo_bytes = (sizeof(FrameGeom) * nf + 15) / 16 * 16, off_bytes = sizeof(int64_t) * (nf + 1);
    const FrameGeom *d_geoms;
    const int64_t *d_offsets;
    const int4 *host_block = nullptr;
    size_t host_block_bytes = 0;
    if (c->staged_in_dev && d_pos == (const double *)c->stage_cur) {
        const size_t at = c->staged_in_dev;
        c->staged_in_dev = 0;
        std::memcpy(c->stage_cur + at, geoms.data(), sizeof(FrameGeom) * nf);
        std::memcpy(c->stage_cur + at + geo_bytes, fr->atom_offsets, off_bytes);
// ... 79 lines not shown
    P.geo_bytes = geo_bytes + off_bytes;
    P.geoms = d_geoms;
    P.frame_of = c->frame_of.as<int>();
    P.spec = c->spec.as<signed char>();
    P.d_offsets = d_offsets;
    P.cl.bin_start = c->bin_start.as<int>(); P.cl.slots = c->slots.as<SlotRec>();
    P.cl.atom_bin = c->atom_bin.as<int>(); P.cl.atom_wrap = c->atom_wrap.as<int>();
    std::memset(&P.n3, 0, sizeof(P.n3));
    if (need_n3 && b->host.T > 0) {
        if (c->n3_cap == 0) c->n3_cap = n3_cap_estimate(b, dens);
        for (int attempt = 0; attempt < 6; attempt++) {
            int cap = c->n3_cap;
            int rc = n3_alloc(c, natoms, cap, P.n3);
            if (rc) return rc;
            HIPCHK(c, hipMemsetAsync(flags + 1, 0, sizeof(int), st));
            size_t lds = (size_t)cap * (8 + 32 + 16);
            if ((int)lds > c->lds_max) return fail(c, UF3_EOVERFLOW, "3-body neighbour list does not fit in LDS");
            const bool block_only = n3_hi >= 0 && !(n3_lo == 0 && n3_hi == natoms) && !uf3_env("UF3_NO_HALO");
            if (!block_only)
                hipLaunchKernelGGL(k_build_n3, dim3(natoms), dim3(64), lds, st, b->dev, P.geoms, P.frame_of, P.cl, P.n3,
                                   d_pos, natoms, flags + 1, 0, (const int *)nullptr, (const int *)nullptr);
            else if (n3_hi > n3_lo) {
                const int nb_ = (int)(n3_hi - n3_lo);
                HIPCHK(c, hipMemsetAsync(P.n3.cnt, 0, sizeof(int) * (size_t)natoms, st));
                hipLaunchKernelGGL(k_build_n3, dim3(nb_), dim3(64), lds, st, b->dev, P.geoms, P.frame_of, P.cl, P.n3,
                                   d_pos, natoms, flags + 1, (int)n3_lo, (const int *)nullptr, (const int *)nullptr);
                int rh = build_halo_lists(b, P, P.n3, d_pos, (int)n3_lo, (int)n3_hi);
                if (rh) return rh;
            }
            HIPCHK(c, hipGetLastError());
            if (defer_check && c->n3_tuned) { P.deferred = true; return UF3_OK; }
            int fl[4] = {0, 0, 0, 0};
            HIPCHK(c, hipMemcpyAsync(fl, flags, sizeof(fl), hipMemcpyDeviceToHost, st));
            HIPCHK(c, hipStreamSynchronize(st));
            if (fl[0]) return check_flags(c);
            const int need = fl[1];
            if (need <= cap) {
                if (!c->n3_tuned) { int rt = n3_tune(c, P.n3, natoms); if (rt) return rt; }
                return UF3_OK;
            }
            c->n3_tuned = true;
            c->n3_cap = (need + 8 + 7) / 8 * 8;
        }
        return fail(c, UF3_EOVERFLOW, "3-body neighbour capacity did not converge");
    }
    return UF3_OK;
}

static int ensure_frag(uf3_ctx *c);

static size_t feat_lds_bytes(int F, int S, int cap, int cand_cap, bool want_e, size_t n_recs, int mode, int dense_stage,
                             int dense_nrec, int n_pair_cols) {
    const bool dense = mode >= 6;
    if (mode == 0) F = S + n_pair_cols;
    size_t e_d = want_e ? (size_t)F + (F & 1) : 0;
    size_t cand_d = (size_t)cand_cap * CAND_STRIDE;
    size_t pair_buf_d = std::max(4 * (size_t)n_pair_cols, (3 * (size_t)cap + 1) / 2 + 2);
    size_t stage_d = mode == 0 ? cand_d + pair_buf_d
                     : (dense ? (size_t)dense_stage : (size_t)NSTAGE * ITEM_STRIDE);
    size_t list_d = mode == 0 ? 0 : 5 * (size_t)cap + ((5 * cap) & 1);
    size_t geo_d = dense ? (size_t)7 * GEO_N : 0;
    size_t per_wave_d = list_d + stage_d + (stage_d & 1) + geo_d;
    size_t per_wave_i = mode == 0 ? 0 : 3 * (size_t)cap + 2 * ((size_t)cap + 1) + (UF3_MAX_SPECIES + 2) +
                                        (size_t)cap * (S + 1);
    size_t ints = ((size_t)WPB * per_wave_i + 3) & ~(size_t)3;
    return (e_d + WPB * per_wave_d) * 8 + ints * 4 + n_recs * sizeof(KnotRec) + 32;
}

static void feat3_shape(const uf3_basis *b, int &ep, int &stage, int &nrec) {
    ep = std::max(3, b->f3_ext_p);
    switch (ep) {
        case 3: stage = F3Cfg<3, 1>::STAGE; nrec = F3Cfg<3, 1>::NREC; break;
        case 4: stage = F3Cfg<4, 2>::STAGE; nrec = F3Cfg<4, 2>::NREC; break;
        case 5: stage = F3Cfg<5, 3>::STAGE; nrec = F3Cfg<5, 3>::NREC; break;
        default: stage = F3Cfg<6, 3>::STAGE; nrec = F3Cfg<6, 3>::NREC; break;
    }
}
static size_t feat3_lds_bytes(const uf3_basis *b, int cap, bool e_lds) {
    int ep, stage, nrec;
    feat3_shape(b, ep, stage, nrec);
    const int F = b->host.F, S = b->host.S;
    const size_t e_d = e_lds ? (size_t)F + (F & 1) : 0, rows_d = (size_t)b->n_f3rows * 18;
    const size_t list_d = 5 * (size_t)cap + ((5 * cap) & 1), tq_d = (size_t)cap * ep * 4, stage_d = (size_t)stage;
    const size_t per_wave_i = 2 * (size_t)cap + 2 * ((size_t)cap + 1) + (UF3_MAX_SPECIES + 2) + (size_t)cap * (S + 1) + 2 * (size_t)nrec + (size_t)cap;
    const size_t ints = ((size_t)WPB * per_wave_i + 3) & ~(size_t)3;
    return (e_d + rows_d + WPB * (list_d + tq_d + stage_d)) * 8 + ints * 4 + (size_t)b->n_f3src * 2 + 32;
}
static size_t feat3w_lds_bytes(const uf3_basis *b, int cap) {
    const size_t rows_d = (size_t)b->n_f3rows * 18;
    const size_t per_wave_d = 8 * (size_t)cap + F3WCfg::STAGE, per_wave_i = 4 * (size_t)cap + (UF3_MAX_SPECIES + 2);
    return (rows_d + WPB * per_wave_d) * 8 + WPB * per_wave_i * 4 + 32;
}
#define UF3_LDS_LIMIT ((size_t)160 * 1024 - 512)

static int featurize_dev_impl(uf3_basis *b, const uf3_frames *fr, const double *d_pos, const int32_t *d_z,
                              double *d_xe, double *d_xf, int64_t ld);

extern "C" int uf3_featurize_dev(uf3_basis *b, const uf3_frames *fr, const double *d_pos, const int32_t *d_z,
                                 double *d_xe, double *d_xf) {
    if (!b) return fail(nullptr, UF3_EINVAL, "null basis");
    return featurize_dev_impl(b, fr, d_pos, d_z, d_xe, d_xf, b->host.F);
}

extern "C" int uf3_featurize_ld_dev(uf3_basis *b, const uf3_frames *fr, const double *d_pos, const int32_t *d_z,
                                    double *d_xe, double *d_xf, int64_t ld) {
    if (!b) return fail(nullptr, UF3_EINVAL, "null basis");
    if (ld < b->host.F || ld > (1 << 24)) return fail(b->ctx, UF3_EINVAL, "uf3_featurize_ld_dev: ld must be >= the number of features");
    return featurize_dev_impl(b, fr, d_pos, d_z, d_xe, d_xf, ld);
}

static int featurize_dev_impl(uf3_basis *b, const uf3_frames *fr, const double *d_pos, const int32_t *d_z,
                              double *d_xe, double *d_xf, int64_t ld) {
    uf3_ctx *c = b->ctx;
    uf3_env_refresh();
    read_f3_env(c);
    if (!d_pos || !d_z) return fail(c, UF3_EINVAL, "null positions / species");
    if (!d_xe && !d_xf) return UF3_OK;
    { int rc0 = poll_pending(c, false, false); if (rc0) return rc0; }
    Prepared P;
    const bool old_n3 = uf3_env("UF3_SEPARATE_N3") != nullptr;
    int rc = prepare(b, fr, d_pos, d_z, old_n3, P);
    if (rc) return rc;
    hipStream_t st = c->stream;
    const int F = b->host.F;
    const bool want_e = d_xe != nullptr, want_f = d_xf != nullptr;
    const bool has3 = b->host.T > 0 && !old_n3;
    if (has3 && c->n3_cap == 0) c->n3_cap = n3_cap_estimate(b, P.max_density);
    int cap = 1;
    auto cand_estimate = [&]() {
        double r = b->host.rsearch;
        double est = P.max_density > 0 ? 4.18879 * r * r * r * P.max_density : 64.0;
        return std::max(32, ((int)(est * 1.6) + 16 + 7) / 8 * 8);
    };
    if (c->cand_cap == 0) c->cand_cap = cand_estimate();
    bool caps_reset = false;
    FeatArgs A;
    A.B = b->dev; A.trios = b->d_trios; A.recs = b->d_recs; A.colsrc = b->d_colsrc;
    A.frag = nullptr;
    A.dense_stage = 0; A.dense_nrec = DENSE_NREC;
    A.dsrc = b->d_dsrc; A.n_dsrc = (int)b->n_dsrc;
    A.gsrc = b->d_gsrc; A.n_gsrc = (int)b->n_gsrc; A.gsrc_lds = 0;
    const int dense_modes = (1 << 6) | (1 << 7) | (1 << 8) | (1 << 9);
    const bool dsrc_ok = (b->modes & dense_modes) && b->n_dsrc * sizeof(int) <= 8192 && !uf3_env("UF3_NO_LDS_DSRC");
    A.dsrc_lds = dsrc_ok;
    if (b->modes & dense_modes) { rc = ensure_frag(c); if (rc) return rc; A.frag = c->frag.as<int>(); }
    A.geoms = P.geoms; A.frame_of = P.frame_of; A.cl = P.cl;
    std::memset(&A.n3, 0, sizeof(A.n3));
    A.n3.cap = 1;
    if (old_n3 && P.n3.cap) A.n3 = P.n3;
    A.build_n3 = has3 ? 1 : 0;
    A.e_direct = (want_e && (size_t)F * 8 > 48 * 1024) ? 1 : 0;
    A.n3_need = c->flags.as<int>() + 1;
    A.n3_seen = nullptr;
    A.pos = d_pos; A.spec = P.spec; A.x_e = d_xe; A.x_f = d_xf; A.ld = (int)ld; A.natoms = P.natoms;
    A.cand_need = c->flags.as<int>() + 2;
    A.outside = uf3_env("UF3_KEEP_GHOST_TERMS") ? nullptr : c->flags.as<int>() + 4;
    { const char *e = uf3_env("UF3_DEBUG_SKIP"); A.skip = e ? atoi(e) : 0; }
    for (int attempt = 0; attempt < 6; attempt++) {
        A.cand_cap = c->cand_cap;
        A.n_recs = (int)b->n_recs;
        A.n_pair_recs = (int)b->n_pair_recs;
        A.trio_rec_lo = (int)b->trio_rec_lo;
        A.wrow_base = (int)(b->wrow_lo * 6); A.n_wrows = b->n_wrows;
        A.n_pair_cols = 0;
        for (int p = 0; p < b->host.P; p++) A.n_pair_cols += b->host.pairs[p].nb;
        if (old_n3) cap = A.n3.cap;
        if (has3) {
            cap = c->n3_cap;
            rc = n3_alloc(c, P.natoms, cap, A.n3);
            if (rc) return rc;
        }
        if (want_e) HIPCHK(c, hipMemsetAsync(d_xe, 0, sizeof(double) * (size_t)P.n_frames * F, st));
        if (!P.flags_zeroed || attempt) HIPCHK(c, hipMemsetAsync(A.n3_need, 0, 2 * sizeof(int), st));
        const bool img_launch = c->img_mode && has3 && want_f && A.outside;
        const bool ext_lists = img_launch;
        if (ext_lists) {
            const int xcap = c->n3x_cap;
            A.n3.xcap = xcap; A.n3.xent = nullptr; A.n3.xoff = nullptr;
            if (xcap > 0) {
                HIPCHK(c, c->n3x_ent.ensure(sizeof(N3Entry) * (size_t)P.natoms * xcap));
                HIPCHK(c, c->n3x_off.ensure(sizeof(int) * (size_t)P.natoms * (UF3_MAX_SPECIES + 1)));
                A.n3.xent = c->n3x_ent.as<N3Entry>(); A.n3.xoff = c->n3x_off.as<int>();
            }
            hipLaunchKernelGGL(k_build_n3_ext, dim3(std::min(P.natoms, 2048)), dim3(64), (size_t)xcap * (8 + 32 + 12) + 16, st,
                               b->dev, P.geoms, P.frame_of, P.cl, A.n3, d_pos, P.natoms, c->flags.as<int>());
        }
        const bool feat3 = b->feat3_ok && want_f && (has3 || old_n3) && !img_launch && cap <= 255 && !c->env_no_feat3 &&
                           feat3_lds_bytes(b, cap, want_e && !A.e_direct) <= UF3_LDS_LIMIT;
        A.n3_seen = nullptr;
        if (feat3 && has3 && cap > 16 && !c->env_f3_no_cap16 && !c->env_f3_no_select) {
            A.n3_seen = c->flags.as<int>() + 7;
            HIPCHK(c, hipMemsetAsync(A.n3_seen, 0, sizeof(int), st));
        }
        bool restart = false;
        {
            Timed tm(c, T_FEAT);
            for (int mode = 0; mode <= 9; mode++) {
                if (!(b->modes & (1 << mode))) continue;
                if (feat3 && mode >= 1) continue;
                const bool dense_mode = mode >= 6;
                const int launch_mode = (mode == 7 && want_f && b->all_grouped7 && !img_launch && !uf3_env("UF3_NO_GROUPED_ONLY")) ? 10
                                        : ((mode == 9 && want_f && b->all_banded9 && !img_launch && !uf3_env("UF3_NO_GROUPED_ONLY")) ? 11 : mode);
                A.trio_rec_lo = (int)(launch_mode == 10 ? b->wrow_lo : b->trio_rec_lo);
                size_t n_rec_mode = mode == 0 ? b->n_pair_recs : b->n_recs - (size_t)A.trio_rec_lo;
                const int S = b->host.S;
                const size_t cu_lds = 160 * 1024 - 1024;
                if (dense_mode) A.dsrc_lds = dsrc_ok && !(mode == 7 && want_f && b->all_grouped7);
                const bool gsrc_wanted = mode == 7 && want_f && b->dense_grouped[7] && b->n_gsrc > 0 && b->n_gsrc * 2 <= 4096 && !uf3_env("UF3_NO_LDS_GSRC");
                const size_t gsrc_bytes = gsrc_wanted ? b->n_gsrc * 2 : 0;
                A.gsrc_lds = gsrc_wanted;
                size_t lds_extra = ((dense_mode && A.dsrc_lds) ? sizeof(int) * b->n_dsrc : 0) + gsrc_bytes;
                bool recs_lds = false;
                size_t lds = 0, lds_plain = 0, lds_recs = 0;
                bool found = false;
                if (dense_mode) {
                    const int stride = want_f ? b->dense_stride_f[mode] : b->dense_stride[mode];
                    const int dump = want_f && b->dense_grouped[mode] ? std::max(768, b->dense_dump[mode]) : b->dense_dump[mode];
                    const bool grouped = want_f && b->dense_grouped[mode];
                    const int nrec_max = std::max(4, std::min(DENSE_NREC, 1200 / stride));
                    auto stage_for = [&](int nr) { return std::max(dump, (nr + (nr & 1) + (grouped ? 2 : 0)) * stride); };
                    A.dense_nrec = nrec_max; A.dense_stage = stage_for(nrec_max);
                    if (mode <= 7 && !uf3_env("UF3_NO_OCC3")) {
                        const int tries[3] = {nrec_max, std::min(nrec_max, 20), std::min(nrec_max, 15)};
                        const size_t budget = (WPB == 4 ? 52 : 13 * WPB) * 1024;
                        const bool dsrc_allowed = A.dsrc_lds, recs_allowed = !uf3_env("UF3_NO_LDS_RECS") && !(img_launch && mode != 0);
                        for (int q = 0; q < 12 && !found; q++) {
                            const int nr = tries[(q % 6) / 2];
                            const bool with_recs = q < 6, with_dsrc = (q & 1) == 0;
                            if ((with_recs && !recs_allowed) || (with_dsrc && !dsrc_allowed)) continue;
                            size_t need = feat_lds_bytes(F, S, cap, A.cand_cap, want_e && !A.e_direct, with_recs ? n_rec_mode : 0, mode,
                                                         stage_for(nr), nr, A.n_pair_cols) + (with_dsrc ? sizeof(int) * b->n_dsrc : 0) + gsrc_bytes;
                            if (need <= budget) {
                                found = true; recs_lds = with_recs; lds = lds_recs = need;
                                A.dense_nrec = nr; A.dense_stage = stage_for(nr); A.dsrc_lds = with_dsrc;
                            }
                        }
                    }
                }
                if (!found) {
                    lds_plain = feat_lds_bytes(F, S, cap, A.cand_cap, want_e && !A.e_direct, 0, mode, A.dense_stage, A.dense_nrec, A.n_pair_cols) + lds_extra;
                    lds_recs = feat_lds_bytes(F, S, cap, A.cand_cap, want_e && !A.e_direct, n_rec_mode, mode, A.dense_stage, A.dense_nrec, A.n_pair_cols) + lds_extra;
                    const size_t lds_target = cu_lds / (mode == 0 ? 4 : 2);
                    recs_lds = lds_recs <= lds_target && !uf3_env("UF3_NO_LDS_RECS") && !(img_launch && mode != 0);
                    lds = recs_lds ? lds_recs : lds_plain;
                }
                if (lds > UF3_LDS_LIMIT && mode == 0 && !c->cand_tuned && c->cand_cap > 64) {
                    while (c->cand_cap > 64 && feat_lds_bytes(F, S, cap, c->cand_cap, want_e && !A.e_direct, recs_lds ? n_rec_mode : 0, 0,
                                                              A.dense_stage, A.dense_nrec, A.n_pair_cols) + lds_extra > UF3_LDS_LIMIT)
                        c->cand_cap = (c->cand_cap * 7 / 8 + 7) / 8 * 8;
                    A.cand_cap = c->cand_cap;
                    lds = feat_lds_bytes(F, S, cap, A.cand_cap, want_e && !A.e_direct, recs_lds ? n_rec_mode : 0, 0, A.dense_stage,
                                         A.dense_nrec, A.n_pair_cols) + lds_extra;
                }
                if (lds > UF3_LDS_LIMIT && !caps_reset) {
                    const int est3 = has3 ? n3_cap_estimate(b, P.max_density) : 0, estc = cand_estimate();
                    if ((has3 && c->n3_cap > est3) || c->cand_cap > estc) {
                        if (has3 && c->n3_cap > est3) { c->n3_cap = est3; c->n3_tuned = false; }
                        if (c->cand_cap > estc) { c->cand_cap = estc; c->cand_tuned = false; }
                        caps_reset = restart = true;
                        break;
                    }
                }
                if (lds > UF3_LDS_LIMIT) return fail(c, UF3_EOVERFLOW, "featurizer LDS footprint exceeds 160 KB (F or neighbour count too large)");
                int per_cu = std::max(1, std::min(8, (int)((size_t)(160 * 1024) / lds)));
                int n_blocks = std::min((P.natoms + WPB - 1) / WPB, c->n_cu * per_cu * 24);
                int apb = ((P.natoms + n_blocks - 1) / n_blocks + WPB - 1) / WPB * WPB;
                n_blocks = (P.natoms + apb - 1) / apb;
                A.atoms_per_block = apb;
                if (uf3_env("UF3_DEBUG_LDS"))
                    fprintf(stderr, "uf3 featurize mode %d: lds %zu B (plain %zu, with recs %zu), recs_lds %d, cap %d, cand_cap %d, "
                            "blocks %d x %d atoms, n_recs %zu, dense nrec %d stage %d\n", launch_mode, lds, lds_plain, lds_recs,
                            (int)recs_lds, cap, A.cand_cap, n_blocks, apb, n_rec_mode, A.dense_nrec, A.dense_stage);
#define UF3_GRID(n) (((n) + 7) / 8 * 8)
 \
#define UF3_LAUNCH1(E, Fo, R, M, I)                                                                                   \
    do {                                                                                                            \
        {                                                                                                           \
            static std::mutex mu; static size_t have[64] = {0};                                                     \
            std::lock_guard<std::mutex> lk(mu);                                                                     \
            size_t &hv = have[c->device & 63];                                                                      \
            if (lds > hv) {                                                                                         \
                HIPCHK(c, hipFuncSetAttribute((const void *)k_featurize<E, Fo, R, M, I>, hipFuncAttributeMaxDynamicSharedMemorySize, (int)lds)); \
                hv = lds;                                                                                           \
            }                                                                                                       \
        }                                                                                                           \
        hipLaunchKernelGGL((k_featurize<E, Fo, R, M, I>), dim3(UF3_GRID(n_blocks)), dim3(WPB * WAVE), lds, st, A);   \
    } while (0)
#define UF3_LAUNCH(M)                                                                                               \
    do {                                                                                                            \
        if (img_launch && M != 0) {          \
            if (want_e) UF3_LAUNCH1(true, true, false, (M == 0 ? 1 : M), true); else UF3_LAUNCH1(false, true, false, (M == 0 ? 1 : M), true); \
        }                                                                                                           \
        else if (want_e && want_f) { if (recs_lds) UF3_LAUNCH1(true, true, true, M, false); else UF3_LAUNCH1(true, true, false, M, false); }   \
        else if (want_f) { if (recs_lds) UF3_LAUNCH1(false, true, true, M, false); else UF3_LAUNCH1(false, true, false, M, false); }    \
        else { if (recs_lds) UF3_LAUNCH1(true, false, true, M, false); else UF3_LAUNCH1(true, false, false, M, false); }               \
    } while (0)
                switch (launch_mode) {
                    case 0: UF3_LAUNCH(0); break;
                    case 1: UF3_LAUNCH(1); break;
                    case 2: UF3_LAUNCH(2); break;
                    case 3: UF3_LAUNCH(3); break;
                    case 4: UF3_LAUNCH(4); break;
                    case 5: UF3_LAUNCH(5); break;
                    case 6: UF3_LAUNCH(6); break;
                    case 7: UF3_LAUNCH(7); break;
                    case 8: UF3_LAUNCH(8); break;
                    case 10: if (want_e) { if (recs_lds) UF3_LAUNCH1(true, true, true, 10, false); else UF3_LAUNCH1(true, true, false, 10, false); }
                             else { if (recs_lds) UF3_LAUNCH1(false, true, true, 10, false); else UF3_LAUNCH1(false, true, false, 10, false); }
                             break;
                    case 11: if (want_e) { if (recs_lds) UF3_LAUNCH1(true, true, true, 11, false); else UF3_LAUNCH1(true, true, false, 11, false); }
                             else { if (recs_lds) UF3_LAUNCH1(false, true, true, 11, false); else UF3_LAUNCH1(false, true, false, 11, false); }
                             break;
                    default: UF3_LAUNCH(9); break;
                }
#undef UF3_LAUNCH
#undef UF3_LAUNCH1
            }
            if (feat3 && !restart) {
                Feat3Args G;
                G.B = b->dev; G.trios = b->d_trios; G.rows = b->d_f3rows; G.n_rows = b->n_f3rows;
                G.fsrc = b->d_f3src; G.trio_fsrc = b->d_f3off; G.n_fsrc = b->n_f3src;
                G.leg_p = b->f3_leg_p; G.leg_n = b->f3_leg_n;
                G.lo_p = b->f3_lo_p; G.ext_p = b->f3_ext_p; G.lo_n = b->f3_lo_n; G.ext_n = b->f3_ext_n;
                G.pr_rows = std::min(b->f3_ext_p, 32 / b->f3_ext_n);
                G.geoms = P.geoms; G.frame_of = P.frame_of; G.n3 = A.n3; G.pos = d_pos; G.spec = P.spec;
                G.x_e = d_xe; G.x_f = d_xf; G.ld = (int)ld; G.natoms = P.natoms; G.e_direct = A.e_direct; G.skip = A.skip;
                G.sel = A.n3_seen; G.sel_mode = 0; G.sel_cap = 16;
                int ep, stage, nrec;
                feat3_shape(b, ep, stage, nrec);
                (void)stage; (void)nrec;
                const int nr = b->f3_nr;
                G.wbuf = nullptr; G.wsz = 0; G.m_lo = 0;
           \
#define UF3_F3_ATTR(KERNEL, lds)                                                                                           \
    do {                                                                                                                   \
        static std::mutex mu; static size_t have[64] = {0};                                                                \
        std::lock_guard<std::mutex> lk(mu);                                                                                \
        size_t &hv = have[c->device & 63];                                                                                 \
        if ((lds) > hv) {                                                                                                  \
            HIPCHK(c, hipFuncSetAttribute((const void *)KERNEL, hipFuncAttributeMaxDynamicSharedMemorySize, (int)(lds)));  \
            hv = (lds);                                                                                                    \
        }                                                                                                                  \
    } while (0)
#define UF3_F3_LAUNCH1(E, EFv, NRv, CAPv, HOv)                                                                              \
    do {                                                                                                                   \
        UF3_F3_ATTR((k_featurize3<E, EFv, NRv, CAPv, HOv>), lds);                                                          \
        hipLaunchKernelGGL((k_featurize3<E, EFv, NRv, CAPv, HOv>), dim3(grid), dim3(WPB * WAVE), lds, st, G);               \
    } while (0)
#define UF3_F3_LAUNCH(E, EFv, NRv)                                                                                          \
    do { if (lcap == 16 && !c->env_f3_no_cap16) UF3_F3_LAUNCH1(E, EFv, NRv, 16, false); else UF3_F3_LAUNCH1(E, EFv, NRv, 0, false); } while (0)
#define UF3_F3W_LAUNCH1(CAPv)                                                                                               \
    do {                                                                                                                   \
        UF3_F3_ATTR((k_feat3_w<3, CAPv>), lds);                                                                            \
        hipLaunchKernelGGL((k_feat3_w<3, CAPv>), dim3(grid), dim3(WPB * WAVE), lds, st, G);                                 \
    } while (0)
                auto f3_grid = [&](size_t lds) -> unsigned {
                    const int n_at = G.natoms - G.m_lo;
                    int per_cu = std::max(1, std::min(8, (int)((size_t)(160 * 1024) / lds)));
                    const int bps = c->env_f3_bps;
                    int n_blocks = std::min((n_at + WPB - 1) / WPB, c->n_cu * per_cu * bps);
                    int apb = ((n_at + n_blocks - 1) / n_blocks + WPB - 1) / WPB * WPB;
                    n_blocks = (n_at + apb - 1) / apb;
                    G.atoms_per_block = apb;
                    return (unsigned)((n_blocks + 7) / 8 * 8);
                };
                auto launch_f3 = [&](int lcap, int sel_mode, bool ho) -> int {
                    G.sel_mode = sel_mode;
                    const size_t lds = feat3_lds_bytes(b, lcap, want_e && !A.e_direct);
                    const unsigned grid = f3_grid(lds);
                    if (c->env_debug_lds)
                        fprintf(stderr, "uf3 featurize3: lds %zu B, cap %d (lists %d apart), selection %d, hand-off %d, blocks %u x %d atoms, window %d x %d, %d round(s)\n",
                                lds, lcap, cap, sel_mode, (int)ho, grid, G.atoms_per_block, G.ext_p, G.ext_n, nr);
                    switch (ep) {
                        case 3:
                            if (ho) {
                                if (lcap == 16 && !c->env_f3_no_cap16) { if (want_e) UF3_F3_LAUNCH1(true, 3, 1, 16, true); else UF3_F3_LAUNCH1(false, 3, 1, 16, true); }
                                else { if (want_e) UF3_F3_LAUNCH1(true, 3, 1, 0, true); else UF3_F3_LAUNCH1(false, 3, 1, 0, true); }
                            }
                            else if ((lcap == 24 || lcap == 32) && !c->env_f3_no_cap16) {
                                if (lcap == 24) { if (want_e) UF3_F3_LAUNCH1(true, 3, 1, 24, false); else UF3_F3_LAUNCH1(false, 3, 1, 24, false); }
                                else { if (want_e) UF3_F3_LAUNCH1(true, 3, 1, 32, false); else UF3_F3_LAUNCH1(false, 3, 1, 32, false); }
                            }
                            else if (want_e) UF3_F3_LAUNCH(true, 3, 1); else UF3_F3_LAUNCH(false, 3, 1);
                            break;
                        case 4: if (want_e) UF3_F3_LAUNCH(true, 4, 2); else UF3_F3_LAUNCH(false, 4, 2); break;
                        case 5: if (want_e) UF3_F3_LAUNCH(true, 5, 3); else UF3_F3_LAUNCH(false, 5, 3); break;
                        default: if (want_e) UF3_F3_LAUNCH(true, 6, 3); else UF3_F3_LAUNCH(false, 6, 3); break;
                    }
                    return UF3_OK;
                };
                auto launch_f3w = [&](int lcap, int sel_mode) -> int {
                    G.sel_mode = sel_mode;
                    const size_t lds = feat3w_lds_bytes(b, lcap);
                    const unsigned grid = f3_grid(lds);
                    if (c->env_debug_lds)
                        fprintf(stderr, "uf3 feat3_w: lds %zu B, cap %d (lists %d apart), selection %d, blocks %u x %d atoms, atoms %d .. %d\n",
                                lds, lcap, cap, sel_mode, grid, G.atoms_per_block, G.m_lo, G.natoms);
                    if (lcap == 16 && !c->env_f3_no_cap16) UF3_F3W_LAUNCH1(16); else UF3_F3W_LAUNCH1(0);
                    return UF3_OK;
                };
                auto launch_pair = [&](bool producer, bool ho) -> int {
                    if (A.n3_seen && cap > 16) {
                        int r1 = producer ? launch_f3w(16, 1) : launch_f3(16, 1, ho);
                        if (r1) return r1;
                        return producer ? launch_f3w(cap, 2) : launch_f3(cap, 2, ho);
                    }
                    return producer ? launch_f3w(cap, 0) : launch_f3(cap, 0, ho);
                };
// ... 1416 lines not shown
extern "C" int uf3_pair_histogram(uf3_basis *b, const uf3_frames *fr, const double *pos, const int32_t *z, int32_t n_bins,
                                  const double *edges, int upper_inclusive, const double *noise, int64_t n_noise, int per_frame,
                                  int64_t *out) {
    uf3_env_refresh();
    if (!b) return fail(nullptr, UF3_EINVAL, "null basis");
    uf3_ctx *c = b->ctx;
    if (!out) return fail(c, UF3_EINVAL, "uf3_pair_histogram: null out");
    if (!fr || fr->n_frames < 1) return fail(c, UF3_EINVAL, "bad uf3_frames");
    if (n_bins < 1) return fail(c, UF3_EINVAL, "uf3_pair_histogram: n_bins must be >= 1");
    int natoms = 0;
    int rc = upload_frames(c, fr, pos, z, natoms);
    if (rc) return rc;
    const size_t n_out = (per_frame ? (size_t)fr->n_frames : 1) * (size_t)b->host.P * (size_t)n_bins;
    HIPCHK(c, c->dbg.ensure(8 * n_out));
    rc = pair_hist_impl(b, fr, (const double *)c->stage_cur, c->d_stage_z, n_bins, edges, upper_inclusive, noise, n_noise,
                        per_frame, c->dbg.as<int64_t>());
    if (rc) return rc;
    HIPCHK(c, hipMemcpyAsync(out, c->dbg.p, 8 * n_out, hipMemcpyDeviceToHost, c->stream));
    HIPCHK(c, hipStreamSynchronize(c->stream));
    c->pin_in_busy = false;
    return check_flags(c);
}

static int neighbors_impl(uf3_basis *b, const uf3_frames *fr, const double *pos, const int32_t *z,
                          int64_t *pair_count, int64_t *pair_ij, double *pair_geo, int64_t pair_cap, int64_t *n3_count,
                          int64_t *n3_ij, int64_t n3_cap) {
    uf3_env_refresh();
    if (!b) return fail(nullptr, UF3_EINVAL, "null basis");
    uf3_ctx *c = b->ctx;
    if (!fr || fr->n_frames != 1) return fail(c, UF3_EINVAL, "the neighbour queries take exactly one frame");
    int natoms = 0;
    int rc = upload_frames(c, fr, pos, z, natoms);
    if (rc) return rc;
    Prepared P;
    rc = prepare(b, fr, (const double *)c->stage_cur, c->d_stage_z, false, P);
    if (rc) return rc;
    int np = b->host.P;
    std::vector<long long> counts(np + 2, 0);
    std::vector<long long> tuples;
    std::vector<double> geo;
    long long cap = 0;
    for (int pass = 0; pass < 2; pass++) {
        const size_t head = 8 * (size_t)(np + 2), ncap = (size_t)std::max<long long>(1, cap);
        HIPCHK(c, c->dbg.ensure(head + 24 * ncap + (pair_geo ? 32 * ncap : 0)));
        long long *d_counts = c->dbg.as<long long>(), *d_tuples = d_counts + np + 2;
        double *d_geo = pair_geo ? (double *)(d_tuples + 3 * ncap) : nullptr;
        HIPCHK(c, hipMemsetAsync(d_counts, 0, head, c->stream));
        hipLaunchKernelGGL(k_debug_pairs, dim3(natoms), dim3(64), 0, c->stream, b->dev, P.geoms, P.frame_of, P.cl,
                           (const double *)c->stage_cur, P.spec, natoms, d_counts, d_tuples, cap, d_geo);
        HIPCHK(c, hipMemcpyAsync(counts.data(), d_counts, head, hipMemcpyDeviceToHost, c->stream));
        HIPCHK(c, hipStreamSynchronize(c->stream));
        if (pass == 0) { cap = counts[np + 1]; if (cap == 0) break; continue; }
        tuples.resize(3 * (size_t)cap);
        HIPCHK(c, hipMemcpy(tuples.data(), d_tuples, 24 * (size_t)cap, hipMemcpyDeviceToHost));
        if (pair_geo) {
            geo.resize(4 * (size_t)cap);
            HIPCHK(c, hipMemcpy(geo.data(), d_geo, 32 * (size_t)cap, hipMemcpyDeviceToHost));
        }
    }
    rc = check_flags(c);
    if (rc) return rc;
    if (pair_count) for (int p = 0; p < np; p++) pair_count[p] = counts[p];
    if (n3_count) *n3_count = counts[np];
    struct T3 { long long p, i, j, at; };
    std::vector<T3> v((size_t)cap);
    for (long long q = 0; q < cap; q++) v[q] = {tuples[3 * q], tuples[3 * q + 1], tuples[3 * q + 2], q};
    std::sort(v.begin(), v.end(), [](const T3 &a, const T3 &bb) {
        return a.p != bb.p ? a.p < bb.p : (a.i != bb.i ? a.i < bb.i : a.j < bb.j);
    });
    std::vector<long long> cur(np + 1, 0);
    for (const T3 &t : v) {
        if (t.p < np) {
            if (cur[t.p] < pair_cap) {
                const long long o = t.p * pair_cap + cur[t.p];
                if (pair_ij) { pair_ij[2 * o] = t.i; pair_ij[2 * o + 1] = t.j; }
                if (pair_geo) for (int k = 0; k < 4; k++) pair_geo[4 * o + k] = geo[4 * (size_t)t.at + k];
            }
        } else if (n3_ij && cur[np] < n3_cap) { n3_ij[2 * cur[np]] = t.i; n3_ij[2 * cur[np] + 1] = t.j; }
        cur[t.p]++;
    }
    return UF3_OK;
}

extern "C" int uf3_n3_lists_debug(uf3_basis *b, int64_t natoms, int64_t *cap_out, int32_t *counts, int32_t *sidx, int64_t sidx_cap) {
    if (!b) return fail(nullptr, UF3_EINVAL, "null basis");
    uf3_ctx *c = b->ctx;
    HIPCHK(c, hipSetDevice(c->device));
    HIPCHK(c, hipStreamSynchronize(c->stream));
    if (c->n3_last_cap <= 0 || natoms != c->n3_last_natoms || !c->n3_cnt.p || !c->n3_dbl.p)
        return fail(c, UF3_EINVAL, "uf3_n3_lists_debug: no 3-body lists of a batch of this size in the workspace");
    const int cap = c->n3_last_cap;
    if (cap_out) *cap_out = cap;
    if (counts) HIPCHK(c, hipMemcpy(counts, c->n3_cnt.p, sizeof(int) * (size_t)natoms, hipMemcpyDeviceToHost));
    if (sidx) {
        if (sidx_cap < cap) return fail(c, UF3_EINVAL, "uf3_n3_lists_debug: sidx_cap below the list capacity");
        std::vector<N3Entry> ent((size_t)natoms * cap);
        HIPCHK(c, hipMemcpy(ent.data(), c->n3_dbl.p, sizeof(N3Entry) * ent.size(), hipMemcpyDeviceToHost));
        for (int64_t a = 0; a < natoms; a++)
            for (int q = 0; q < cap; q++) sidx[a * sidx_cap + q] = ent[(size_t)a * cap + q].sidx;
    }
    return UF3_OK;
}

extern "C" int uf3_neighbors_debug(uf3_basis *b, const uf3_frames *fr, const double *pos, const int32_t *z,
                                   int64_t *pair_count, int64_t *pair_ij, int64_t pair_cap, int64_t *n3_count,
                                   int64_t *n3_ij, int64_t n3_cap) {
    return neighbors_impl(b, fr, pos, z, pair_count, pair_ij, nullptr, pair_cap, n3_count, n3_ij, n3_cap);
}

extern "C" int uf3_pair_geometry(uf3_basis *b, const uf3_frames *fr, const double *pos, const int32_t *z,
                                 int64_t *pair_count, int64_t *pair_ij, double *pair_geo, int64_t pair_cap) {
    if (pair_cap > 0 && !pair_geo) return fail(b ? b->ctx : nullptr, UF3_EINVAL, "uf3_pair_geometry: null pair_geo");
    return neighbors_impl(b, fr, pos, z, pair_count, pair_ij, pair_cap > 0 ? pair_geo : nullptr, pair_cap, nullptr, nullptr, 0);
}

extern "C" int uf3_distance_matrix(uf3_ctx *c, const double *a, int64_t na, const double *bb, int64_t nb, double *out) {
    if (!c) return fail(nullptr, UF3_EINVAL, "null ctx");
    if (na < 0 || nb < 0 || (na && !a) || (nb && !bb)) return fail(c, UF3_EINVAL, "uf3_distance_matrix: bad argument");
    const size_t n = (size_t)na * (size_t)nb;
    if (!n) return UF3_OK;
    if (!out) return fail(c, UF3_EINVAL, "uf3_distance_matrix: null out");
    HIPCHK(c, hipSetDevice(c->device));
    HIPCHK(c, c->dbg.ensure(24 * (size_t)(na + nb) + 8 * n));
    double *d_a = c->dbg.as<double>(), *d_b = d_a + 3 * na, *d_out = d_b + 3 * nb;
    HIPCHK(c, hipMemcpyAsync(d_a, a, 24 * (size_t)na, hipMemcpyHostToDevice, c->stream));
    HIPCHK(c, hipMemcpyAsync(d_b, bb, 24 * (size_t)nb, hipMemcpyHostToDevice, c->stream));
    hipLaunchKernelGGL(k_distance_matrix, dim3((unsigned)((n + 255) / 256)), dim3(256), 0, c->stream, d_a, (long long)na, d_b,
                       (long long)nb, d_out);
    HIPCHK(c, hipGetLastError());
    HIPCHK(c, hipMemcpyAsync(out, d_out, 8 * n, hipMemcpyDeviceToHost, c->stream));
    HIPCHK(c, hipStreamSynchronize(c->stream));
    return UF3_OK;
}

extern "C" int uf3_direction_cosines(uf3_ctx *c, const double *sup_pos, int64_t n_sup, const int64_t *i_where,
                                     const int64_t *j_where, const double *rij, int64_t n_d, int64_t n_atoms, double *out) {
    if (!c) return fail(nullptr, UF3_EINVAL, "null ctx");
    if (n_sup < 0 || n_d < 0 || n_atoms < 0) return fail(c, UF3_EINVAL, "uf3_direction_cosines: bad argument");
    const size_t n = (size_t)n_atoms * 3 * (size_t)n_d;
    if (!n) return UF3_OK;
    if (!sup_pos || !i_where || !j_where || !rij || !out) return fail(c, UF3_EINVAL, "uf3_direction_cosines: null argument");
    for (int64_t q = 0; q < n_d; q++)
        if (i_where[q] < 0 || i_where[q] >= n_sup || j_where[q] < 0 || j_where[q] >= n_sup)
            return fail(c, UF3_EINVAL, "uf3_direction_cosines: index outside the supercell");
    HIPCHK(c, hipSetDevice(c->device));
    HIPCHK(c, c->dbg.ensure(24 * (size_t)n_sup + 24 * (size_t)n_d + 8 * n));
    double *d_pos = c->dbg.as<double>();
    long long *d_i = (long long *)(d_pos + 3 * n_sup), *d_j = d_i + n_d;
    double *d_r = (double *)(d_j + n_d), *d_out = d_r + n_d;
    HIPCHK(c, hipMemcpyAsync(d_pos, sup_pos, 24 * (size_t)n_sup, hipMemcpyHostToDevice, c->stream));
    HIPCHK(c, hipMemcpyAsync(d_i, i_where, 8 * (size_t)n_d, hipMemcpyHostToDevice, c->stream));
    HIPCHK(c, hipMemcpyAsync(d_j, j_where, 8 * (size_t)n_d, hipMemcpyHostToDevice, c->stream));
    HIPCHK(c, hipMemcpyAsync(d_r, rij, 8 * (size_t)n_d, hipMemcpyHostToDevice, c->stream));
    hipLaunchKernelGGL(k_direction_cosines, dim3((unsigned)((n + 255) / 256)), dim3(256), 0, c->stream, d_pos, d_i, d_j, d_r,
                       (long long)n_d, (long long)n_atoms, d_out);
    HIPCHK(c, hipGetLastError());
    HIPCHK(c, hipMemcpyAsync(out, d_out, 8 * n, hipMemcpyDeviceToHost, c->stream));
    HIPCHK(c, hipStreamSynchronize(c->stream));
    return UF3_OK;
}

#ifdef UF3_PHASE_TIMING
extern "C" int uf3_debug_phase(unsigned long long *out16) {
    hipDeviceSynchronize();
    hipMemcpyFromSymbol(out16, HIP_SYMBOL(g_phase), sizeof(unsigned long long) * 16);
    unsigned long long z[16] = {0};
// ... 5 lines not shown
```

### uf3_amd/csrc/uf3_kernels.h

```cpp
#pragma once
#include "uf3_device.h"

__global__ void k_frame_bins(const BasisDev *B, const FrameGeom *geoms, const int64_t *atom_offsets,
                             int n_frames, int natoms, const double *pos, const int32_t *z,
                             int *frame_of, int *atom_bin, int *atom_wrap, signed char *spec,
                             int *sort_key, int *bin_count, int *err_flag) {
    int a = blockIdx.x * blockDim.x + threadIdx.x;
    if (a >= natoms) return;
    int lo = 0, hi = n_frames - 1;
    while (lo < hi) {
        int mid = (lo + hi + 1) >> 1;
        if (atom_offsets[mid] <= a) lo = mid; else hi = mid - 1;
    }
    const FrameGeom &g = geoms[lo];
    frame_of[a] = lo;
    int zz = z[a];
    int s = (zz >= 0 && zz < 120) ? B->z2s[zz] : -1;
    if (s < 0) { atomicExch(err_flag, 2); s = 0; }
    spec[a] = (signed char)s;
    double x = pos[3 * (size_t)a], y = pos[3 * (size_t)a + 1], w = pos[3 * (size_t)a + 2];
    int bin[3], wrap[3];
    bool far_out = false;
    for (int k = 0; k < 3; k++) {
        double f = x * g.inv[k] + y * g.inv[3 + k] + w * g.inv[6 + k];
// ... 512 lines not shown
    if (s0 == 0 && s1 == 0 && s2 == 0) return m_local < ksidx;
    int k0, k1, k2;
    unpack3(kshift, k0, k1, k2);
    bool k_real = (k0 + s0 == 0) && (k1 + s1 == 0) && (k2 + s2 == 0);
    return k_real ? (m_local < k_local) : true;
}

#ifndef WPB
#define WPB 4
#endif
#define NSTAGE 32
#define CAND_STRIDE 6
#define ITEM_STRIDE 38

#ifdef UF3_ABLATE
#define UF3_SKIP(bit) (A.skip & (bit))
#else
#define UF3_SKIP(bit) 0
#endif

#ifdef UF3_PHASE_TIMING
__device__ unsigned long long g_phase[16];
struct PhaseClock {
    unsigned long long t;
    __device__ __forceinline__ PhaseClock() : t(__builtin_amdgcn_s_memtime()) {}
    __device__ __forceinline__ void lap(int phase) {
        asm volatile("s_waitcnt vmcnt(0) lgkmcnt(0)" ::: "memory");
        unsigned long long n = __builtin_amdgcn_s_memtime();
        if (lane_id() == 0) atomicAdd(&g_phase[phase], n - t);
        t = __builtin_amdgcn_s_memtime();
    }
};
#else
struct PhaseClock { __device__ __forceinline__ void lap(int) {} };
#endif

template <class T>
__device__ __forceinline__ T load_const(const T *p) {
    static_assert(sizeof(T) % sizeof(int) == 0, "word-sized tables only");
    typedef const __attribute__((address_space(4))) int *ConstInts;
    ConstInts src = (ConstInts)(unsigned long long)p;
    T out;
    int *dst = (int *)&out;
#pragma unroll
    for (int q = 0; q < (int)(sizeof(T) / sizeof(int)); q++) dst[q] = src[q];
    return out;
}

struct FeatArgs {
    const BasisDev *B;
    const TrioDev *trios;
    const KnotRec *recs;
    const int *colsrc;
    const int *frag;
    const int *dsrc;
    int n_dsrc, dsrc_lds;
    const unsigned short *gsrc;
    int n_gsrc, gsrc_lds;
    const FrameGeom *geoms;
    const int *frame_of;
    CellList cl;
    N3Lists n3;
    const double *pos;
    const signed char *spec;
    double *x_e;
    double *x_f;
    int ld;
    int *cand_need;
    const int *outside;
    int *n3_need;
    int *n3_seen;
    int build_n3;
    int e_direct;
    int natoms, atoms_per_block;
    int cand_cap;
    int n_recs;
    int n_pair_recs;
    int wrow_base, n_wrows;
    int trio_rec_lo;
    int n_pair_cols;
    int dense_stage;
    int dense_nrec;
    int skip;
};

__device__ __forceinline__ void lds_add(double *p, double v) {
    __hip_atomic_fetch_add(p, v, __ATOMIC_RELAXED, __HIP_MEMORY_SCOPE_WORKGROUP);
}
__device__ __forceinline__ void wave_sync() {
    __builtin_amdgcn_fence(__ATOMIC_ACQ_REL, "wavefront");
    __builtin_amdgcn_wave_barrier();
}

struct ESink {
    double *lds;
    double *glob;
    bool direct;
    __device__ __forceinline__ void add(int col, double v) const {
        if (v == 0.0) return;
        if (direct) unsafeAtomicAdd(glob + col, v); else lds_add(lds + col, v);
    }
};

struct TripletGeom {
    double rl, rm, rn;
    double a1[3], a2[3], a3[3];
    bool centre;
    bool first;
    int i1, i2;
};

struct TripletRec {
    double v[3][4], d[3][4];
    int first[3];
};

template <bool WANT_F>
__device__ __forceinline__ bool eval_triplet(const KnotRec *recs, const TrioDev *td, const TripletGeom &t, bool valid,
                                             TripletRec &r) {
    if (!valid) return false;
    if (!((t.rl > td->leg[0].t0) && (t.rl < td->leg[0].tlast) && (t.rm > td->leg[1].t0) && (t.rm < td->leg[1].tlast) &&
          (t.rn > td->leg[2].t0) && (t.rn < td->leg[2].tlast))) return false;
    KnotRec kl, km, kn;
    int il = load_interval(recs, td->leg[0], t.rl, kl);
    int im = load_interval(recs, td->leg[1], t.rm, km);
    int in = load_interval(recs, td->leg[2], t.rn, kn);
    bspline4<WANT_F>(kl, t.rl, r.v[0], r.d[0]);
    bspline4<WANT_F>(km, t.rm, r.v[1], r.d[1]);
    bspline4<WANT_F>(kn, t.rn, r.v[2], r.d[2]);
    r.first[0] = il - 3; r.first[1] = im - 3; r.first[2] = in - 3;
    return true;
}

struct ColSrc { int l, m, n; };

template <bool WANT_E, bool WANT_F, int NSRC, int NCH>
__device__ __forceinline__ void gather_one(const double *rec, const ColSrc (&src)[NCH][NSRC], double (&acc)[NCH][4]) {
    const int4 mt = *(const int4 *)(rec + 34);
    double2 a01 = {0, 0}, a23 = {0, 0}, a45 = {0, 0}, a67 = {0, 0};
    double a8 = 0.0;
    if (WANT_F) {
        a01 = *(const double2 *)(rec + 24); a23 = *(const double2 *)(rec + 26);
        a45 = *(const double2 *)(rec + 28); a67 = *(const double2 *)(rec + 30);
        a8 = rec[32];
    }
    const bool centre = WANT_E && mt.w != 0;
#pragma unroll
    for (int ch = 0; ch < NCH; ch++) {
#pragma unroll
        for (int k = 0; k < NSRC; k++) {
            const unsigned a = (unsigned)(src[ch][k].l - mt.x), b = (unsigned)(src[ch][k].m - mt.y),
                           c = (unsigned)(src[ch][k].n - mt.z);
            const bool ok = (a | b | c) < 4u;
            const double2 L = *(const double2 *)(rec + 2 * (a & 3u));
            const double2 M = *(const double2 *)(rec + 8 + 2 * (b & 3u));
            const double2 N = *(const double2 *)(rec + (ok ? 16 + 2 * (c & 3u) : 36));
            const double z = L.x * M.x;
            if (centre) acc[ch][3] = fma(z, N.x, acc[ch][3]);
            if (WANT_F) {
                const double p1 = L.y * (M.x * N.x), p2 = M.y * (L.x * N.x), p3 = N.y * z;
                acc[ch][0] = fma(p3, a67.x, fma(p2, a23.y, fma(p1, a01.x, acc[ch][0])));
                acc[ch][1] = fma(p3, a67.y, fma(p2, a45.x, fma(p1, a01.y, acc[ch][1])));
                acc[ch][2] = fma(p3, a8, fma(p2, a45.y, fma(p1, a23.x, acc[ch][2])));
            }
        }
    }
// ... 1135 lines not shown
            if (!(d > p_rmin && d < p_rmax)) continue;
            KnotRec kr;
            double v[4], dv[4];
            const int first = load_interval<RL ? 3 : 1>(recs, leg, d, kr) - 3;
            bspline4<WANT_F>(kr, d, v, dv);
            const double s = 2.0 / d;
            const double dir[3] = {s * c[0], s * c[1], s * c[2]};
            const int hi = p_nb - trail2, base = p_col - S;
#pragma unroll
            for (int q = 0; q < 4; q++) {
                const int bf = first + q;
                if (bf >= lead2 && bf < hi) {
                    double *dst = row + base + bf;
                    if (WANT_E) lds_add(dst, v[q]);
                    if (WANT_F) { lds_add(dst + n2, dv[q] * dir[0]); lds_add(dst + 2 * n2, dv[q] * dir[1]); lds_add(dst + 3 * n2, dv[q] * dir[2]); }
                }
            }
        }
    }
    wave_sync();
    for (int col = lane; col < n2; col += WAVE) {
        if (WANT_F) {
            double *dst = A.x_f + (size_t)m * 3 * A.ld + S + col;
            __builtin_nontemporal_store(row[n2 + col], dst); __builtin_nontemporal_store(row[2 * n2 + col], dst + A.ld);
            __builtin_nontemporal_store(row[3 * n2 + col], dst + 2 * (size_t)A.ld);
        }
        if (WANT_E) es.add(S + col, row[col]);
    }
    wave_sync();
}

__device__ __forceinline__ void build_n3_list(const FeatArgs &A, const BasisDev *B, const FrameGeom &g, const WaveLds &w,
                                              int m, int n_cand) {
    const int lane = lane_id(), cap = A.n3.cap;
    unsigned long long *key = (unsigned long long *)w.pstage;
    int *src = (int *)(key + cap);
    const double rmin3 = load_const(&B->rmin3), rmax3 = load_const(&B->rmax3);
    int count = 0;
    for (int e0 = 0; e0 < n_cand; e0 += WAVE) {
        const int e = e0 + lane;
        const double *c = w.cand + (size_t)e * CAND_STRIDE;
        const bool ok = e < n_cand && c[3] > rmin3 && c[3] <= rmax3;
        const unsigned long long mask = __ballot(ok);
        if (ok) {
            const int slot = count + mbcnt(mask);
            if (slot < cap) {
                const int2 ps = *(const int2 *)(c + 5);
                int s0, s1, s2;
                unpack3(ps.y, s0, s1, s2);
                const int sidx = supercell_index(g, s0, s1, s2, ps.x - g.atom_lo);
                key[slot] = ((unsigned long long)(int)c[4] << 32) | (unsigned)sidx;
                src[slot] = e;
            }
        }
        count += __popcll(mask);
    }
    wave_sync();
    if (A.n3_seen && lane == 0 && count > __builtin_nontemporal_load(A.n3_seen)) atomicMax(A.n3_seen, count);
    if (count > cap) { if (lane == 0) atomicMax(A.n3_need, count); count = cap; }
    if (lane == 0) A.n3.cnt[m] = count;
    if (count <= WAVE) {
        const int my_spec = lane < count ? (int)(key[lane] >> 32) : UF3_MAX_SPECIES;
        int below = count;
        for (int sp = 0; sp <= load_const(&B->S); sp++) {
            const int n_lower = __popcll(__ballot(my_spec < sp));
            if (lane == sp) below = n_lower;
        }
        if (lane <= UF3_MAX_SPECIES) A.n3.spoff[(size_t)m * (UF3_MAX_SPECIES + 1) + lane] = below;
    } else
        for (int sp = lane; sp <= UF3_MAX_SPECIES; sp += WAVE) {
            int below = 0;
            for (int f = 0; f < count; f++) below += (int)(key[f] >> 32) < sp;
            A.n3.spoff[(size_t)m * (UF3_MAX_SPECIES + 1) + sp] = below;
        }
    for (int e = lane; e < count; e += WAVE) {
        const unsigned long long k = key[e];
        int rank = 0;
        for (int f = 0; f < count; f++) rank += key[f] < k;
        const double *c = w.cand + (size_t)src[e] * CAND_STRIDE;
        const int2 ps = *(const int2 *)(c + 5);
        N3Entry out;
        out.dx = c[0]; out.dy = c[1]; out.dz = c[2]; out.r = c[3];
        out.parent = ps.x; out.shiftc = ps.y; out.sidx = (int)(unsigned)k; out.spec = (int)(k >> 32);
        A.n3.ent[(size_t)m * cap + rank] = out;
    }
    wave_sync();
}

__device__ __forceinline__ void zero_rows(double *x_f, int m, int ld, int col, int n) {
    for (int c = lane_id(); c < n; c += WAVE) {
        double *dst = x_f + (size_t)m * 3 * ld + col + c;
        __builtin_nontemporal_store(0.0, dst); __builtin_nontemporal_store(0.0, dst + ld); __builtin_nontemporal_store(0.0, dst + 2 * (size_t)ld);
    }
}

__device__ __forceinline__ int trio_mode(const TrioDev *td) {
    if (td->dense) return td->dense;
    const bool wide = td->ncol > WAVE;
    return td->nsrc == 1 ? (wide ? 2 : 1) : (td->nsrc == 2 ? (wide ? 4 : 3) : 5);
}

template <bool WANT_E, bool WANT_F, bool RECS_LDS, int MODE_, bool IMG>
__global__ void __launch_bounds__(WPB * WAVE, MODE_ == 0 ? 5 : ((MODE_ == 6 || MODE_ == 7 || MODE_ == 10) ? 3 : 2))
k_featurize(FeatArgs A) {
    constexpr int MODE = MODE_ == 10 ? 7 : (MODE_ == 11 ? 9 : MODE_);
    constexpr bool GROUPED_ONLY = MODE_ == 10 || MODE_ == 11;
    extern __shared__ __align__(16) unsigned char smem[];
    const BasisDev *B = A.B;
    const int F = load_const(&B->F), S = load_const(&B->S), n_trios = load_const(&B->T), cap = A.n3.cap;
    if (!IMG && WANT_F && MODE != 0 && A.outside && A.outside[0]) return;
    const int tid = threadIdx.x, lane = tid & 63;
    const int wave = __builtin_amdgcn_readfirstlane(tid >> 6);
    double *erow = (double *)smem;
    const bool e_lds = WANT_E && !A.e_direct;
    const int FE = MODE == 0 ? S + A.n_pair_cols : F;
    const size_t e_d = e_lds ? (size_t)FE + (FE & 1) : 0;
    const size_t cand_d = (size_t)A.cand_cap * CAND_STRIDE;
    const size_t pair_buf_d = max(4 * (size_t)A.n_pair_cols, (3 * (size_t)cap + 1) / 2 + 2);
    constexpr bool DENSE = MODE >= 6;
    const size_t stage_d = MODE == 0 ? cand_d + pair_buf_d
                           : (DENSE ? (size_t)A.dense_stage : (size_t)NSTAGE * ITEM_STRIDE);
    const size_t list_d = MODE == 0 ? 0 : 5 * (size_t)cap + ((5 * cap) & 1);
    const size_t geo_d = DENSE ? (size_t)7 * GEO_N : 0;
    const size_t per_wave_d = list_d + stage_d + (stage_d & 1) + geo_d;
    const size_t per_wave_i = MODE == 0 ? 0 : 3 * (size_t)cap + 2 * ((size_t)cap + 1) + (UF3_MAX_SPECIES + 2) +
                                                  (size_t)cap * (S + 1);
    double *wd = erow + e_d + (size_t)wave * per_wave_d;
    int *wi = (int *)(erow + e_d + (size_t)WPB * per_wave_d) + (size_t)wave * per_wave_i;
    WaveLds w;
    w.ox = wd; w.oy = w.ox + cap; w.oz = w.oy + cap; w.orr = w.oz + cap; w.oir = w.orr + cap;
    w.stage = wd + list_d;
    w.geo = w.stage + stage_d + (stage_d & 1);
    w.cand = w.stage;
    w.pstage = w.stage + cand_d;
    w.oparent = wi; w.oshift = wi + cap; w.osidx = wi + 2 * cap;
    w.noff = wi + 3 * cap; w.nbase = w.noff + cap + 1; w.so = w.nbase + cap + 1;
    w.ospoff = w.so + (UF3_MAX_SPECIES + 2);
    w.sp_stride = S + 1;

    KnotRec *recs_lds;
    {
        size_t ints_total = ((size_t)WPB * per_wave_i + 3) & ~(size_t)3;
        recs_lds = (KnotRec *)((int *)(erow + e_d + (size_t)WPB * per_wave_d) + ints_total);
    }
    const int rec_first = MODE == 0 ? 0 : A.trio_rec_lo, rec_end = MODE == 0 ? A.n_pair_recs : A.n_recs;
    if (RECS_LDS) {
        const double *srcp = (const double *)(A.recs + rec_first);
        double *dstp = (double *)recs_lds;
        for (int q = tid; q < (rec_end - rec_first) * 12; q += WPB * WAVE) dstp[q] = srcp[q];
    }
    const KnotRec *recs = RECS_LDS ? recs_lds - rec_first : A.recs;
    int fragp[4] = {0, 0, 0, 0};
    const int *dsrc = A.dsrc;
    const unsigned short *gsrc = A.gsrc;
    if (DENSE) {
        for (int v = 0; v < 4; v++) fragp[v] = A.frag[(lane * 4 + v) * 2] * 16 + A.frag[(lane * 4 + v) * 2 + 1];
        int *dl = (int *)(recs_lds + (RECS_LDS ? rec_end - rec_first : 0));
        if (A.dsrc_lds) {
            for (int q = tid; q < A.n_dsrc; q += WPB * WAVE) dl[q] = A.dsrc[q];
            dsrc = dl;
            dl += A.n_dsrc;
        }
        if (A.gsrc_lds) {
            for (int q = tid; q < A.n_gsrc / 2; q += WPB * WAVE) dl[q] = ((const int *)A.gsrc)[q];
            gsrc = (const unsigned short *)dl;
        }
    }
// ... 1616 lines not shown
```

Before: 6409.

## Precompute per-bond spline values at neighbor-list build and reuse in 3-body featurizer

Evaluates each n3 bond's pair-leg spline values and sub-block index once, at neighbor-list construction or in a new k_f3_bonds kernel, and stores them in a new global buffer. The featurizer's neighbor-of-neighbor loop can then read these records instead of re-evaluating the spline per triple. That loop is also restructured to walk per-wave chunks of centres, dropping the noff/nbase LDS prefix arrays and the binary search. The cost is extra global memory traffic and a bond buffer sized natoms*cap, plus a debug export.

```diff
diff --git a/include/uf3_hip.h b/include/uf3_hip.h
--- a/include/uf3_hip.h
+++ b/include/uf3_hip.h
@@ -141,6 +141,7 @@
                         int64_t *pair_count, int64_t *pair_ij, int64_t pair_cap,
                         int64_t *n3_count, int64_t *n3_ij, int64_t n3_cap);
 int uf3_n3_lists_debug(uf3_basis *basis, int64_t natoms, int64_t *cap_out, int32_t *counts, int32_t *sidx, int64_t sidx_cap);
+int uf3_n3_bonds_debug(uf3_basis *basis, int64_t natoms, int64_t *cap_out, double *r, double *bv, int32_t *bsb, int32_t *window);
 
 int uf3_pair_geometry(uf3_basis *basis, const uf3_frames *frame, const double *pos, const int32_t *z,
                       int64_t *pair_count, int64_t *pair_ij, double *pair_geo, int64_t pair_cap);
diff --git a/uf3_amd/_lib.py b/uf3_amd/_lib.py
--- a/uf3_amd/_lib.py
+++ b/uf3_amd/_lib.py
@@ -16,7 +16,7 @@
            "uf3_featurize", "uf3_featurize_dev", "uf3_gram", "uf3_gram_dev",
            "uf3_eval", "uf3_eval_dev", "uf3_eval_virial", "uf3_eval_virial_dev", "uf3_eval_atoms", "uf3_eval_atoms_dev",
            "uf3_eval_centres", "uf3_eval_centres_dev",
-           "uf3_neighbors_debug", "uf3_n3_lists_debug", "uf3_fit_rows_dev", "uf3_fit_pack_dev", "uf3_gram_force_rows_dev",
+           "uf3_neighbors_debug", "uf3_n3_lists_debug", "uf3_n3_bonds_debug", "uf3_fit_rows_dev", "uf3_fit_pack_dev", "uf3_gram_force_rows_dev",
            "uf3_pair_geometry", "uf3_distance_matrix", "uf3_direction_cosines",
            "uf3_ctx_md_skin", "uf3_ctx_md_stats",
            "uf3_featurize_ld_dev", "uf3_fit_create", "uf3_fit_destroy", "uf3_fit_reset", "uf3_fit_add", "uf3_fit_pack", "uf3_fit_info", "uf3_fit_use_flat", "uf3_fit_first_chunk",
@@ -157,6 +157,7 @@
             getattr(lib, name).argtypes = [vp, C.POINTER(Frames), vp, vp, vp, vp, vp, i64, i64, vp, vp, vp]
         lib.uf3_neighbors_debug.argtypes = [vp, C.POINTER(Frames), vp, vp, vp, vp, i64, vp, vp, i64]
         lib.uf3_n3_lists_debug.argtypes = [vp, i64, vp, vp, vp, i64]
+        lib.uf3_n3_bonds_debug.argtypes = [vp, i64, vp, vp, vp, vp, vp]
         lib.uf3_gram_force_rows_dev.argtypes = [vp, vp, vp, vp, i64, i64, i32, vp, vp]
         lib.uf3_pair_geometry.argtypes = [vp, C.POINTER(Frames), vp, vp, vp, vp, vp, i64]
         lib.uf3_distance_matrix.argtypes = [vp, vp, i64, vp, i64, vp]
diff --git a/uf3_amd/csrc/uf3_device.h b/uf3_amd/csrc/uf3_device.h
--- a/uf3_amd/csrc/uf3_device.h
+++ b/uf3_amd/csrc/uf3_device.h
@@ -118,6 +118,8 @@
     int xcap;
     int *xoff;
     N3Entry *xent;
+    double *bv;
+    int *bsb;
 };
 
 __device__ __forceinline__ int pack3(int a, int b, int c) { return (a + 512) | ((b + 512) << 10) | ((c + 512) << 20); }
@@ -347,3 +349,71 @@
         }
     }
 }
+
+struct Feat3Leg {
+    double t0, tlast, inv_h;
+    int nk, row0;
+};
+
+typedef double __attribute__((ext_vector_type(2))) F3Pair;
+typedef const __attribute__((address_space(3))) F3Pair *F3LdsPairs;
+typedef const __attribute__((address_space(3))) double *F3LdsDoubles;
+
+#ifndef F3_ROWS_GLOBAL
+#define F3_ROWS_GLOBAL 0
+#endif
+typedef const __attribute__((address_space(1))) F3Pair *F3GlobalPairs;
+template <bool DERIV, bool GLOBAL = F3_ROWS_GLOBAL>
+__device__ __forceinline__ int f3_eval(const double *rows, const Feat3Leg &lg, double x, double (&v)[4], double (&d)[4]) {
+    const int hi = lg.nk - 5;
+    int iv = 3 + (int)((x - lg.t0) * lg.inv_h);
+    iv = iv < 3 ? 3 : (iv > hi ? hi : iv);
+    F3Pair kn, cf[8];
+    auto load_row = [&](int i) {
+        F3Pair t0, t[8];
+        if (GLOBAL) {
+            F3GlobalPairs q = (F3GlobalPairs)(const F3Pair *)(rows + (size_t)(lg.row0 + i - 3) * 18);
+            t0 = q[0];
+#pragma unroll
+            for (int e = 0; e < 8; e++) t[e] = q[1 + e];
+        } else {
+            F3LdsPairs q = (F3LdsPairs)(const F3Pair *)(rows + (size_t)(lg.row0 + i - 3) * 18);
+            t0 = q[0];
+#pragma unroll
+            for (int e = 0; e < 8; e++) t[e] = q[1 + e];
+        }
+        kn = t0;
+#pragma unroll
+        for (int e = 0; e < 8; e++) cf[e] = t[e];
+        __builtin_amdgcn_sched_group_barrier(GLOBAL ? 0x020 : 0x100, 9, 0);
+    };
+    load_row(iv);
+    if (__builtin_expect(x > kn.y && iv < hi, 0)) {
+        do { ++iv; load_row(iv); } while (x > kn.y && iv < hi);
+    } else if (__builtin_expect(x <= kn.x && iv > 3, 0)) {
+        do { --iv; load_row(iv); } while (x <= kn.x && iv > 3);
+    }
+    const double u = x - kn.x;
+#pragma unroll
+    for (int fq = 0; fq < 4; fq++) {
+        const double c0 = cf[2 * fq].x, c1 = cf[2 * fq].y, c2 = cf[2 * fq + 1].x, c3 = cf[2 * fq + 1].y;
+        double pv = fma(c3, u, c2), pd = fma(c3, u, pv);
+        pv = fma(pv, u, c1); pd = fma(pd, u, pv);
+        pv = fma(pv, u, c0);
+        v[fq] = pv;
+        if (DERIV) d[fq] = pd;
+    }
+    return iv;
+}
+
+__device__ __forceinline__ void f3_bond_record(const double *rows, const Feat3Leg &lg, int lo, int sb_max, double r, double *bv,
+                                               int *bsb) {
+    double v[4] = {0, 0, 0, 0}, d[4];
+    int sb = 0;
+    if (r > lg.t0 && r < lg.tlast) {
+        const int iv = f3_eval<false, true>(rows, lg, r, v, d);
+        sb = max(0, min(sb_max, iv - 3 - lo));
+    }
+    *(double2 *)bv = double2{v[0], v[1]}; *(double2 *)(bv + 2) = double2{v[2], v[3]};
+    if (bsb) *bsb = sb;
+}
diff --git a/uf3_amd/csrc/uf3_feat3.h b/uf3_amd/csrc/uf3_feat3.h
--- a/uf3_amd/csrc/uf3_feat3.h
+++ b/uf3_amd/csrc/uf3_feat3.h
@@ -1,9 +1,5 @@
 #pragma once
 
-struct Feat3Leg {
-    double t0, tlast, inv_h;
-    int nk, row0;
-};
 
 struct Feat3Args {
     const BasisDev *B;
@@ -45,51 +41,13 @@
     static constexpr int MIN_WAVES = NR == 1 ? 4 : 2;
 };
 
-typedef double __attribute__((ext_vector_type(2))) F3Pair;
-typedef const __attribute__((address_space(3))) F3Pair *F3LdsPairs;
-typedef const __attribute__((address_space(3))) double *F3LdsDoubles;
-
-#ifndef F3_ROWS_GLOBAL
-#define F3_ROWS_GLOBAL 0
-#endif
-typedef const __attribute__((address_space(1))) F3Pair *F3GlobalPairs;
-template <bool DERIV>
-__device__ __forceinline__ int f3_eval(const double *rows, const Feat3Leg &lg, double x, double (&v)[4], double (&d)[4]) {
-    const int hi = lg.nk - 5;
-    int iv = 3 + (int)((x - lg.t0) * lg.inv_h);
-    iv = iv < 3 ? 3 : (iv > hi ? hi : iv);
-    F3Pair kn, cf[8];
-    auto load_row = [&](int i) {
-#if F3_ROWS_GLOBAL
-        F3GlobalPairs q = (F3GlobalPairs)(const F3Pair *)(rows + (size_t)(lg.row0 + i - 3) * 18);
-#else
-        F3LdsPairs q = (F3LdsPairs)(const F3Pair *)(rows + (size_t)(lg.row0 + i - 3) * 18);
-#endif
-        F3Pair t0 = q[0], t[8];
-#pragma unroll
-        for (int e = 0; e < 8; e++) t[e] = q[1 + e];
-        kn = t0;
-#pragma unroll
-        for (int e = 0; e < 8; e++) cf[e] = t[e];
-        __builtin_amdgcn_sched_group_barrier(F3_ROWS_GLOBAL ? 0x020 : 0x100, 9, 0);
-    };
-    load_row(iv);
-    if (__builtin_expect(x > kn.y && iv < hi, 0)) {
-        do { ++iv; load_row(iv); } while (x > kn.y && iv < hi);
-    } else if (__builtin_expect(x <= kn.x && iv > 3, 0)) {
-        do { --iv; load_row(iv); } while (x <= kn.x && iv > 3);
-    }
-    const double u = x - kn.x;
-#pragma unroll
-    for (int fq = 0; fq < 4; fq++) {
-        const double c0 = cf[2 * fq].x, c1 = cf[2 * fq].y, c2 = cf[2 * fq + 1].x, c3 = cf[2 * fq + 1].y;
-        double pv = fma(c3, u, c2), pd = fma(c3, u, pv);
-        pv = fma(pv, u, c1); pd = fma(pd, u, pv);
-        pv = fma(pv, u, c0);
-        v[fq] = pv;
-        if (DERIV) d[fq] = pd;
-    }
-    return iv;
+__global__ void __launch_bounds__(256)
+k_f3_bonds(N3Lists n3, const double *rows, Feat3Leg lg, int lo, int sb_max, int natoms) {
+    const size_t s = (size_t)blockIdx.x * 256 + threadIdx.x;
+    if (s >= (size_t)natoms * n3.cap) return;
+    const int m = (int)(s / n3.cap), e = (int)(s - (size_t)m * n3.cap);
+    if (e >= n3.cnt[m]) return;
+    f3_bond_record(rows, lg, lo, sb_max, n3.ent[s].r, n3.bv + 4 * s, n3.bsb ? n3.bsb + s : nullptr);
 }
 
 #ifndef F3_WIDE_MINW
@@ -120,14 +78,14 @@
     const size_t list_d = 5 * (size_t)cap + ((5 * cap) & 1), tq_d = (size_t)cap * EF * 4;
     constexpr size_t stage_d = Cfg::STAGE;
     const size_t per_wave_d = list_d + tq_d + stage_d;
-    const size_t per_wave_i = 2 * (size_t)cap + 2 * ((size_t)cap + 1) + (UF3_MAX_SPECIES + 2) + (size_t)cap * (S + 1) + 2 * NREC + cap;
+    const size_t per_wave_i = 2 * (size_t)cap + (UF3_MAX_SPECIES + 2) + (size_t)cap * (S + 1) + 2 * NREC + cap;
     double *wd = rows_lds + rows_d + (size_t)wave * per_wave_d;
     int *wi = (int *)(rows_lds + rows_d + (size_t)WPB * per_wave_d) + (size_t)wave * per_wave_i;
     double *ox = wd, *oy = ox + cap, *oz = oy + cap, *orr = oz + cap, *oir = orr + cap;
     double *tq = wd + list_d;
     double *stage = tq + tq_d;
     double *zq = stage + (Cfg::STAGE - 4);
-    int *oparent = wi, *oshift = wi + cap, *noff = wi + 2 * cap, *nbase = noff + cap + 1, *so = nbase + cap + 1;
+    int *oparent = wi, *oshift = wi + cap, *so = wi + 2 * cap;
     int *osbp = so + (UF3_MAX_SPECIES + 2);
     int *hdrs = osbp + cap;
     int *ospoff = hdrs + 2 * NREC;
@@ -192,11 +150,32 @@
         const int n_own = load_const(A.n3.cnt + m);
         wave_sync();
         for (int e = lane; e < n_own; e += WAVE) {
-            const N3Entry en = A.n3.ent[(size_t)m * ent_stride + e];
-            ox[e] = en.dx; oy[e] = en.dy; oz[e] = en.dz; orr[e] = en.r; oir[e] = 1.0 / en.r;
+            const size_t s = (size_t)m * ent_stride + e;
+            const N3Entry en = A.n3.ent[s];
+            double v[4] = {0, 0, 0, 0}, d[4] = {0, 0, 0, 0};
+            int sbp = 0;
+            if (en.r > leg_p.t0 && en.r < leg_p.tlast && !UF3_SKIP(32)) {
+                const int iv = f3_eval<true>(rows, leg_p, en.r, v, d);
+                sbp = max(0, min(sbp_max, iv - 3 - lo_p));
+            }
+            const double ir = 1.0 / en.r;
+            ox[e] = en.dx; oy[e] = en.dy; oz[e] = en.dz; orr[e] = en.r; oir[e] = ir;
             int s0, s1, s2;
             unpack3(en.shiftc, s0, s1, s2);
             oparent[e] = en.parent; oshift[e] = pack3(-s0, -s1, -s2);
+            if (EF > 4) osbp[e] = sbp;
+            const double ux = en.dx * ir, uy = en.dy * ir, uz = en.dz * ir;
+            double *dst = tq + (size_t)e * EF * 4;
+            if (EF > 4) {
+#pragma unroll
+                for (int q = 0; q < EF; q++) { *(double2 *)(dst + 4 * q) = double2{0.0, 0.0}; *(double2 *)(dst + 4 * q + 2) = double2{0.0, 0.0}; }
+                dst += 4 * sbp;
+            }
+#pragma unroll
+            for (int q = 0; q < (EF < 4 ? EF : 4); q++) {
+                *(double2 *)(dst + 4 * q) = double2{ux * d[q], uy * d[q]};
+                *(double2 *)(dst + 4 * q + 2) = double2{uz * d[q], v[q]};
+            }
         }
         if (lane <= S) so[lane] = A.n3.spoff[(size_t)m * (UF3_MAX_SPECIES + 1) + lane];
         wave_sync();
@@ -205,28 +184,6 @@
                 const int *src = A.n3.spoff + (size_t)oparent[e] * (UF3_MAX_SPECIES + 1);
                 for (int sp = 0; sp <= S; sp++) ospoff[e * (S + 1) + sp] = src[sp];
             }
-        for (int e = lane; e < n_own; e += WAVE) {
-            const double r = orr[e];
-            double v[4] = {0, 0, 0, 0}, d[4] = {0, 0, 0, 0};
-            int sbp = 0;
-            if (r > leg_p.t0 && r < leg_p.tlast && !UF3_SKIP(32)) {
-                const int iv = f3_eval<true>(rows, leg_p, r, v, d);
-                sbp = max(0, min(sbp_max, iv - 3 - lo_p));
-            }
-            if (EF > 4) osbp[e] = sbp;
-            const double ir = oir[e], ux = ox[e] * ir, uy = oy[e] * ir, uz = oz[e] * ir;
-            double *dst = tq + (size_t)e * EF * 4;
-            if (EF > 4) {
-#pragma unroll
-                for (int q = 0; q < EF; q++) { *(double2 *)(dst + 4 * q) = double2{0.0, 0.0}; *(double2 *)(dst + 4 * q + 2) = double2{0.0, 0.0}; }
-                dst += 4 * sbp;
-            }
-#pragma unroll
-            for (int q = 0; q < (EF < 4 ? EF : 4); q++) {
-                *(double2 *)(dst + 4 * q) = double2{ux * d[q], uy * d[q]};
-                *(double2 *)(dst + 4 * q + 2) = double2{uz * d[q], v[q]};
-            }
-        }
         wave_sync();
 
         for (int t = 0; t < n_trios; t++) {
@@ -387,120 +344,126 @@
             if (!HO && nbr && !UF3_SKIP(8)) {
                 const int sx = sm == t_sa ? t_sb : t_sa;
                 const int rc_lo = so[t_sc], ncen = so[t_sc + 1] - rc_lo;
-                int total_n = 0;
-                for (int e0 = 0; e0 < ncen; e0 += WAVE) {
-                    const int e = e0 + lane;
-                    int cnt = 0, base = 0;
-                    if (e < ncen) {
-                        const int *sp = ospoff + (size_t)(rc_lo + e) * sp_stride;
-                        base = sp[sx]; cnt = sp[sx + 1] - base;
-                    }
-                    const int incl = wave_scan_incl(cnt);
-                    if (e < ncen) { noff[e] = total_n + incl - cnt; nbase[e] = base; }
-                    total_n += __builtin_amdgcn_readlane(incl, WAVE - 1);
-                }
-                total_n = __builtin_amdgcn_readfirstlane(total_n);
-                if (lane == 0) noff[ncen] = total_n;
-                wave_sync();
-                for (int p0 = 0; p0 < total_n; p0 += WAVE) {
-                    const int q = p0 + lane;
-                    bool valid = q < total_n;
-                    double pv[4] = {0, 0, 0, 0}, bn[4] = {0, 0, 0, 0}, bd[4] = {0, 0, 0, 0}, a3[3] = {0, 0, 0}, dum[4];
-                    int sbn = 0, sbp = 0, e = 0;
-                    if (valid) {
-                        int lo = 0, hi = ncen - 1;
-                        while (lo < hi) { const int mid = (lo + hi + 1) >> 1; if (noff[mid] <= q) lo = mid; else hi = mid - 1; }
-                        e = rc_lo + lo;
-                        const int kk = nbase[lo] + (q - noff[lo]);
-                        const int pc = oparent[e];
-                        const double oex = ox[e], oey = oy[e], oez = oz[e], oer = orr[e];
-                        const N3Entry ke = A.n3.ent[(size_t)pc * ent_stride + kk];
-                        valid = !(ke.parent == m && ke.shiftc == oshift[e]);
-                        const double ex = oex + ke.dx, ey = oey + ke.dy, ez = oez + ke.dz;
-                        const double rn = norm3_leg(ex, ey, ez), rk = ke.r;
-                        valid = valid & (oer > leg_p.t0) & (oer < leg_p.tlast) & (rk > leg_p.t0) & (rk < leg_p.tlast) &
-                                (rn > leg_n.t0) & (rn < leg_n.tlast);
-                        if (valid && !UF3_SKIP(64)) {
-                            const double in = fast_rcp(rn);
-                            a3[0] = ex * in; a3[1] = ey * in; a3[2] = ez * in;
-                            const int ivp = f3_eval<false>(rows, leg_p, rk, pv, dum);
-                            sbp = max(0, min(sbp_max, ivp - 3 - lo_p));
-                            const int iv = f3_eval<true>(rows, leg_n, rn, bn, bd);
-                            sbn = max(0, min(sbn_max, iv - 3 - lo_n));
-                        }
-                    }
-                    const unsigned long long mask = __ballot(valid);
-                    const int nv = __popcll(mask), rank = mbcnt(mask);
-                    int smask = (1 << NR) - 1;
-                    if (EF > 4) {
-                        const int rm = valid ? rounds_of(sbp) : 0;
-                        smask = 0;
-#pragma unroll
-                        for (int r = 0; r < NR; r++) smask |= __ballot((rm >> r) & 1) ? (1 << r) : 0;
-                    }
-                    for (int sp0 = 0; sp0 < nv; sp0 += NREC) {
-                        const int slot = rank - sp0;
-                        if (valid && slot >= 0 && slot < NREC) {
-                            double *rp = stage + (size_t)slot * RS_N;
-                            if (EF > 4) {
-#pragma unroll
-                                for (int u = 0; u < EFP; u += 2) *(double2 *)(rp + u) = double2{0.0, 0.0};
-#pragma unroll
-                                for (int u = 0; u < 4; u++) rp[sbp + u] = pv[u];
-                            } else {
-                                *(double2 *)rp = double2{pv[0], pv[1]};
-                                *(double2 *)(rp + 2) = double2{pv[2], pv[3]};
+                for (int c0 = 0; c0 < ncen; c0 += WAVE) {
+                    int rlen = 0, base = 0;
+                    if (c0 + lane < ncen) {
+                        const int *sp = ospoff + (size_t)(rc_lo + c0 + lane) * sp_stride;
+                        base = sp[sx]; rlen = sp[sx + 1] - base;
+                    }
+                    const int incl = wave_scan_incl(rlen);
+                    const int total_n = __builtin_amdgcn_readlane(incl, WAVE - 1);
+                    const int kb = base - (incl - rlen);
+                    const unsigned long long nonempty = __ballot(rlen > 0);
+                    const unsigned long long behind = lane < WAVE - 1 ? nonempty >> (lane + 1) : 0ull;
+                    const int next_ne = behind ? lane + 1 + __builtin_ctzll(behind) : WAVE;
+                    for (int p0 = 0; p0 < total_n; p0 += WAVE) {
+                        const int q = p0 + lane;
+                        bool valid = q < total_n;
+                        const int pe = incl - p0;
+                        const bool sender = (rlen > 0) & (pe > 0) & (pe < WAVE);
+                        const int got = __builtin_amdgcn_ds_permute((sender ? pe : 0) << 2, sender ? next_ne + 1 : 0);
+                        const unsigned long long holds = __ballot((rlen > 0) & (pe > 0));
+                        const int first = holds ? __builtin_ctzll(holds) : 0;
+                        const int reached = wave_scan_max(lane == 0 ? 0 : got);
+                        const int run = min(reached ? reached - 1 : first, WAVE - 1);
+                        const int kk = __shfl(kb, run) + q;
+                        double pv[4] = {0, 0, 0, 0}, bn[4] = {0, 0, 0, 0}, bd[4] = {0, 0, 0, 0}, a3[3] = {0, 0, 0};
+                        int sbn = 0, sbp = 0, e = 0;
+                        if (valid) {
+                            e = rc_lo + c0 + run;
+                            const int pc = oparent[e];
+                            const double oex = ox[e], oey = oy[e], oez = oz[e], oer = orr[e];
+                            const size_t ks = (size_t)pc * ent_stride + kk;
+                            const N3Entry ke = A.n3.ent[ks];
+                            const F3Pair p01 = *(const F3Pair *)(A.n3.bv + 4 * ks), p23 = *(const F3Pair *)(A.n3.bv + 4 * ks + 2);
+                            const int ksb = EF > 4 ? A.n3.bsb[ks] : 0;
+                            valid = !(ke.parent == m && ke.shiftc == oshift[e]);
+                            const double ex = oex + ke.dx, ey = oey + ke.dy, ez = oez + ke.dz;
+                            const double rn = norm3_leg(ex, ey, ez), rk = ke.r;
+                            valid = valid & (oer > leg_p.t0) & (oer < leg_p.tlast) & (rk > leg_p.t0) & (rk < leg_p.tlast) &
+                                    (rn > leg_n.t0) & (rn < leg_n.tlast);
+                            if (valid && !UF3_SKIP(64)) {
+                                const double in = fast_rcp(rn);
+                                a3[0] = ex * in; a3[1] = ey * in; a3[2] = ez * in;
+                                pv[0] = p01.x; pv[1] = p01.y; pv[2] = p23.x; pv[3] = p23.y;
+                                sbp = ksb;
+                                const int iv = f3_eval<true>(rows, leg_n, rn, bn, bd);
+                                sbn = max(0, min(sbn_max, iv - 3 - lo_n));
                             }
-#pragma unroll
-                            for (int u = 0; u < 4; u++) {
-                                *(double2 *)(rp + EFP + 4 * u) = double2{a3[0] * bd[u], a3[1] * bd[u]};
-                                *(double2 *)(rp + EFP + 2 + 4 * u) = double2{a3[2] * bd[u], bn[u]};
+                        }
+                        const unsigned long long mask = __ballot(valid);
+                        const int nv = __popcll(mask), rank = mbcnt(mask);
+                        int smask = (1 << NR) - 1;
+                        if (EF > 4) {
+                            const int rm = valid ? rounds_of(sbp) : 0;
+                            smask = 0;
+#pragma unroll
+                            for (int r = 0; r < NR; r++) smask |= __ballot((rm >> r) & 1) ? (1 << r) : 0;
+                        }
+                        for (int sp0 = 0; sp0 < nv; sp0 += NREC) {
+                            const int slot = rank - sp0;
+                            if (valid && slot >= 0 && slot < NREC) {
+                                double *rp = stage + (size_t)slot * RS_N;
+                                if (EF > 4) {
+#pragma unroll
+                                    for (int u = 0; u < EFP; u += 2) *(double2 *)(rp + u) = double2{0.0, 0.0};
+#pragma unroll
+                                    for (int u = 0; u < 4; u++) rp[sbp + u] = pv[u];
+                                } else {
+                                    *(double2 *)rp = double2{pv[0], pv[1]};
+                                    *(double2 *)(rp + 2) = double2{pv[2], pv[3]};
+                                }
+#pragma unroll
+                                for (int u = 0; u < 4; u++) {
+                                    *(double2 *)(rp + EFP + 4 * u) = double2{a3[0] * bd[u], a3[1] * bd[u]};
+                                    *(double2 *)(rp + EFP + 2 + 4 * u) = double2{a3[2] * bd[u], bn[u]};
+                                }
+                                hdrs[slot] = e; hdrs[NREC + slot] = sbn * 32;
                             }
-                            hdrs[slot] = e; hdrs[NREC + slot] = sbn * 32;
-                        }
-                        wave_sync();
-                        const int r_end = min(NREC, nv - sp0);
-                        const int v_key = hdrs[min(lane, NREC - 1)], v_prev = hdrs[min(max(lane - 1, 0), NREC - 1)];
-                        unsigned long long gm = __ballot(lane < r_end && (lane == 0 || v_key != v_prev));
-                        while (gm && !UF3_SKIP(1)) {
-                            const int g0 = __builtin_ctzll(gm);
-                            gm &= gm - 1;
-                            const int g1 = gm ? __builtin_ctzll(gm) : r_end;
-                            const int key = __builtin_amdgcn_readlane(v_key, g0);
-                            if (key != cur) { flush(false); cur = key; }
-                            wmask |= smask;
-                            const double *rp = stage + (size_t)g0 * RS_N;
-                            const int *sp = hdrs + NREC + g0;
-                            int cnt = g1 - g0;
-                            auto body = [&](auto tag) {
-                                constexpr int CNT = decltype(tag)::value;
-                                int sb[CNT];
-#pragma unroll
-                                for (int i = 0; i < CNT; i++) sb[i] = ((const __attribute__((address_space(3))) int *)sp)[i];
-#pragma unroll
-                                for (int r = 0; r < NR; r++) {
-                                    if (EF > 4 && !((smask >> r) & 1)) continue;
-                                    double bq[CNT];
-                                    F3Pair tt[CNT];
-#pragma unroll
-                                    for (int i = 0; i < CNT; i++) {
-                                        const unsigned off = (unsigned)(n32_lane[r] - sb[i]);
-                                        const char *qa = (const char *)(rp + i * RS_N + EFP + 2 * half) + off;
-                                        qa = off < 128u ? qa : (const char *)zq;
-                                        bq[i] = ((F3LdsDoubles)rp)[i * RS_N + p_lane[r]];
-                                        tt[i] = *(F3LdsPairs)(const F3Pair *)qa;
+                            wave_sync();
+                            const int r_end = min(NREC, nv - sp0);
+                            const int v_key = hdrs[min(lane, NREC - 1)], v_prev = hdrs[min(max(lane - 1, 0), NREC - 1)];
+                            unsigned long long gm = __ballot(lane < r_end && (lane == 0 || v_key != v_prev));
+                            while (gm && !UF3_SKIP(1)) {
+                                const int g0 = __builtin_ctzll(gm);
+                                gm &= gm - 1;
+                                const int g1 = gm ? __builtin_ctzll(gm) : r_end;
+                                const int key = __builtin_amdgcn_readlane(v_key, g0);
+                                if (key != cur) { flush(false); cur = key; }
+                                wmask |= smask;
+                                const double *rp = stage + (size_t)g0 * RS_N;
+                                const int *sp = hdrs + NREC + g0;
+                                int cnt = g1 - g0;
+                                auto body = [&](auto tag) {
+                                    constexpr int CNT = decltype(tag)::value;
+                                    int sb[CNT];
+#pragma unroll
+                                    for (int i = 0; i < CNT; i++) sb[i] = ((const __attribute__((address_space(3))) int *)sp)[i];
+#pragma unroll
+                                    for (int r = 0; r < NR; r++) {
+                                        if (EF > 4 && !((smask >> r) & 1)) continue;
+                                        double bq[CNT];
+                                        F3Pair tt[CNT];
+#pragma unroll
+                                        for (int i = 0; i < CNT; i++) {
+                                            const unsigned off = (unsigned)(n32_lane[r] - sb[i]);
+                                            const char *qa = (const char *)(rp + i * RS_N + EFP + 2 * half) + off;
+                                            qa = off < 128u ? qa : (const char *)zq;
+                                            bq[i] = ((F3LdsDoubles)rp)[i * RS_N + p_lane[r]];
+                                            tt[i] = *(F3LdsPairs)(const F3Pair *)qa;
+                                        }
+#pragma unroll
+                                        for (int i = 0; i < CNT; i++) { ws[r][0] = fma(bq[i], tt[i].x, ws[r][0]); ws[r][1] = fma(bq[i], tt[i].y, ws[r][1]); }
                                     }
-#pragma unroll
-                                    for (int i = 0; i < CNT; i++) { ws[r][0] = fma(bq[i], tt[i].x, ws[r][0]); ws[r][1] = fma(bq[i], tt[i].y, ws[r][1]); }
-                                }
-                                rp += CNT * RS_N; sp += CNT; cnt -= CNT;
-                            };
-                            while (cnt >= 4) body(std::integral_constant<int, 4>{});
-                            if (cnt == 3) body(std::integral_constant<int, 3>{});
-                            else if (cnt == 2) body(std::integral_constant<int, 2>{});
-                            else if (cnt == 1) body(std::integral_constant<int, 1>{});
-                        }
-                        wave_sync();
+                                    rp += CNT * RS_N; sp += CNT; cnt -= CNT;
+                                };
+                                while (cnt >= 4) body(std::integral_constant<int, 4>{});
+                                if (cnt == 3) body(std::integral_constant<int, 3>{});
+                                else if (cnt == 2) body(std::integral_constant<int, 2>{});
+                                else if (cnt == 1) body(std::integral_constant<int, 1>{});
+                            }
+                            wave_sync();
+                        }
                     }
                 }
                 flush(false);
diff --git a/uf3_amd/csrc/uf3_hip.hip b/uf3_amd/csrc/uf3_hip.hip
--- a/uf3_amd/csrc/uf3_hip.hip
+++ b/uf3_amd/csrc/uf3_hip.hip
@@ -76,10 +76,12 @@
         bin_cnt,
         part_sums,
         hist_edges, hist_noise,
-        f3w;
+        f3w,
+        n3_bond;
     int n3_cap = 0, cand_cap = 0;
     size_t bin_cnt_clean = 0;
     int n3_last_cap = 0, n3_last_natoms = 0;
+    bool n3_last_bonds = false;
     int n3x_cap = 0;
     bool img_mode = false;
     int gram_plan_np[UF3_MAX_SPECIES + 1] = {0}, gram_plan_blocks[UF3_MAX_SPECIES + 1] = {0}, gram_plan_next = 0;
@@ -280,7 +282,7 @@
     Buf *all[] = {&c->geoms, &c->offsets, &c->frame_of, &c->atom_bin, &c->atom_wrap, &c->spec, &c->key_in,
                   &c->key_out, &c->val_in, &c->val_out, &c->sort_tmp, &c->bin_start, &c->slots, &c->flags, &c->n3_cnt, &c->n3_int, &c->n3_dbl, &c->e_atom, &c->nbr_f, &c->coeff,
                   &c->stage_pos, &c->stage_z, &c->stage_out, &c->stage_out2, &c->sp_rows, &c->sp_seg, &c->gram_tij, &c->frag, &c->dbg, &c->halo, &c->n3x_ent, &c->n3x_off,
-                  &c->bin_cnt, &c->f3w, &c->coeff_cw, &c->part_sums};
+                  &c->bin_cnt, &c->f3w, &c->n3_bond, &c->coeff_cw, &c->part_sums};
     for (Buf *b : all) b->release();
     for (Buf &b : c->gram_tiles) b.release();
     if (c->comm) uf3_comm_destroy(c);
@@ -1069,7 +1071,7 @@
     HIPCHK(c, c->n3_cnt.ensure(sizeof(int) * (size_t)natoms * (UF3_MAX_SPECIES + 2)));
     HIPCHK(c, c->n3_dbl.ensure(sizeof(N3Entry) * (size_t)natoms * cap));
     n3.cap = cap;
-    c->n3_last_cap = cap; c->n3_last_natoms = natoms;
+    c->n3_last_cap = cap; c->n3_last_natoms = natoms; c->n3_last_bonds = false;
     n3.cnt = c->n3_cnt.as<int>();
     n3.spoff = n3.cnt + natoms;
     n3.ent = c->n3_dbl.as<N3Entry>();
@@ -1315,7 +1317,7 @@
     const int F = b->host.F, S = b->host.S;
     const size_t e_d = e_lds ? (size_t)F + (F & 1) : 0, rows_d = (size_t)b->n_f3rows * 18;
     const size_t list_d = 5 * (size_t)cap + ((5 * cap) & 1), tq_d = (size_t)cap * ep * 4, stage_d = (size_t)stage;
-    const size_t per_wave_i = 2 * (size_t)cap + 2 * ((size_t)cap + 1) + (UF3_MAX_SPECIES + 2) + (size_t)cap * (S + 1) + 2 * (size_t)nrec + (size_t)cap;
+    const size_t per_wave_i = 2 * (size_t)cap + (UF3_MAX_SPECIES + 2) + (size_t)cap * (S + 1) + 2 * (size_t)nrec + (size_t)cap;
     const size_t ints = ((size_t)WPB * per_wave_i + 3) & ~(size_t)3;
     return (e_d + rows_d + WPB * (list_d + tq_d + stage_d)) * 8 + ints * 4 + (size_t)b->n_f3src * 2 + 32;
 }
@@ -1420,6 +1422,15 @@
         }
         const bool feat3 = b->feat3_ok && want_f && (has3 || old_n3) && !img_launch && cap <= 255 && !c->env_no_feat3 &&
                            feat3_lds_bytes(b, cap, want_e && !A.e_direct) <= UF3_LDS_LIMIT;
+        A.n3.bv = nullptr; A.n3.bsb = nullptr;
+        A.f3rows = b->d_f3rows; A.f3leg = b->f3_leg_p; A.f3_lo = b->f3_lo_p; A.f3_sbmax = std::max(0, b->f3_ext_p - 4);
+        if (feat3) {
+            const size_t slots = (size_t)P.natoms * cap;
+            HIPCHK(c, c->n3_bond.ensure(slots * (4 * sizeof(double) + (A.f3_sbmax > 0 ? sizeof(int) : 0))));
+            A.n3.bv = c->n3_bond.as<double>();
+            if (A.f3_sbmax > 0) A.n3.bsb = (int *)(A.n3.bv + 4 * slots);
+        }
+        c->n3_last_bonds = feat3;
         A.n3_seen = nullptr;
         if (feat3 && has3 && cap > 16 && !c->env_f3_no_cap16 && !c->env_f3_no_select) {
             A.n3_seen = c->flags.as<int>() + 7;
@@ -1557,6 +1568,11 @@
                 G.lo_p = b->f3_lo_p; G.ext_p = b->f3_ext_p; G.lo_n = b->f3_lo_n; G.ext_n = b->f3_ext_n;
                 G.pr_rows = std::min(b->f3_ext_p, 32 / b->f3_ext_n);
                 G.geoms = P.geoms; G.frame_of = P.frame_of; G.n3 = A.n3; G.pos = d_pos; G.spec = P.spec;
+                if (!has3) {
+                    const size_t slots = (size_t)P.natoms * cap;
+                    hipLaunchKernelGGL(k_f3_bonds, dim3((unsigned)((slots + 255) / 256)), dim3(256), 0, st, A.n3, A.f3rows, A.f3leg,
+                                       A.f3_lo, A.f3_sbmax, P.natoms);
+                }
                 G.x_e = d_xe; G.x_f = d_xf; G.ld = (int)ld; G.natoms = P.natoms; G.e_direct = A.e_direct; G.skip = A.skip;
                 G.sel = A.n3_seen; G.sel_mode = 0; G.sel_cap = 16;
                 int ep, stage, nrec;
@@ -3139,6 +3155,32 @@
     return UF3_OK;
 }
 
+extern "C" int uf3_n3_bonds_debug(uf3_basis *b, int64_t natoms, int64_t *cap_out, double *r, double *bv, int32_t *bsb,
+                                  int32_t *window) {
+    if (!b) return fail(nullptr, UF3_EINVAL, "null basis");
+    uf3_ctx *c = b->ctx;
+    HIPCHK(c, hipSetDevice(c->device));
+    HIPCHK(c, hipStreamSynchronize(c->stream));
+    if (c->n3_last_cap <= 0 || natoms != c->n3_last_natoms || !c->n3_last_bonds || !c->n3_bond.p)
+        return fail(c, UF3_EINVAL, "uf3_n3_bonds_debug: no bond records of a batch of this size in the workspace");
+    const int cap = c->n3_last_cap;
+    const size_t slots = (size_t)natoms * cap;
+    if (cap_out) *cap_out = cap;
+    if (window) { window[0] = b->f3_lo_p; window[1] = b->f3_ext_p; }
+    if (r) {
+        std::vector<N3Entry> ent(slots);
+        HIPCHK(c, hipMemcpy(ent.data(), c->n3_dbl.p, sizeof(N3Entry) * slots, hipMemcpyDeviceToHost));
+        for (size_t s = 0; s < slots; s++) r[s] = ent[s].r;
+    }
+    const double *d_bv = c->n3_bond.as<double>();
+    if (bv) HIPCHK(c, hipMemcpy(bv, d_bv, sizeof(double) * 4 * slots, hipMemcpyDeviceToHost));
+    if (bsb) {
+        if (b->f3_ext_p > 4) HIPCHK(c, hipMemcpy(bsb, d_bv + 4 * slots, sizeof(int) * slots, hipMemcpyDeviceToHost));
+        else std::memset(bsb, 0, sizeof(int) * slots);
+    }
+    return UF3_OK;
+}
+
 extern "C" int uf3_n3_lists_debug(uf3_basis *b, int64_t natoms, int64_t *cap_out, int32_t *counts, int32_t *sidx, int64_t sidx_cap) {
     if (!b) return fail(nullptr, UF3_EINVAL, "null basis");
     uf3_ctx *c = b->ctx;
diff --git a/uf3_amd/csrc/uf3_kernels.h b/uf3_amd/csrc/uf3_kernels.h
--- a/uf3_amd/csrc/uf3_kernels.h
+++ b/uf3_amd/csrc/uf3_kernels.h
@@ -618,6 +618,9 @@
     int dense_stage;
     int dense_nrec;
     int skip;
+    const double *f3rows;
+    Feat3Leg f3leg;
+    int f3_lo, f3_sbmax;
 };
 
 __device__ __forceinline__ void lds_add(double *p, double v) {
@@ -1919,7 +1922,9 @@
         N3Entry out;
         out.dx = c[0]; out.dy = c[1]; out.dz = c[2]; out.r = c[3];
         out.parent = ps.x; out.shiftc = ps.y; out.sidx = (int)(unsigned)k; out.spec = (int)(k >> 32);
-        A.n3.ent[(size_t)m * cap + rank] = out;
+        const size_t slot = (size_t)m * cap + rank;
+        A.n3.ent[slot] = out;
+        if (A.n3.bv) f3_bond_record(A.f3rows, A.f3leg, A.f3_lo, A.f3_sbmax, out.r, A.n3.bv + 4 * slot, A.n3.bsb ? A.n3.bsb + slot : nullptr);
     }
     wave_sync();
 }
```

Result: faster. 6551, median of 6 (+2.2%).
